# cokwa/bitHTM

Measured on AMD Instinct MI355X. Metric: HTM timesteps/sec (SP + TM, learning on), 65536 cols x 32 cells, higher is better.
Workload: dtype u32 bit-packed / f64 + f32 permanences; 1 GPU; configs[2]: 65536 columns x 32 cells, SP + TM learning on, 1 MI355X; input_dim=1024, column_dim=65536, cell_dim=32, active_columns=1311, patterns=50, pretrain_steps=500, segments=96476, segment_slots=128, hip_graph=True, hip_graph_requested=True, pipelined=True, repetitions=15, streamed_calls=True

## Files before the change

bithtm_amd/_lib.py:

```python

import ctypes as C
import os

HERE = os.path.dirname(os.path.abspath(__file__))
LIB_PATH = os.path.join(HERE, "libbithtm_hip.so")
ABI_VERSION = 4


class HtmConfig(C.Structure):
    _fields_ = [
        ("struct_bytes", C.c_uint32), ("device", C.c_int32),
        ("input_dim", C.c_int32), ("column_dim", C.c_int32), ("cell_dim", C.c_int32),
        ("active_columns", C.c_int32), ("enable_sp", C.c_int32), ("enable_tm", C.c_int32),
        ("sp_permanence_threshold", C.c_double), ("sp_delta_on", C.c_double), ("sp_delta_off", C.c_double),
        ("boost_coefficient", C.c_float), ("duty_momentum", C.c_float), ("duty_increment", C.c_float),
        ("tm_learn_active", C.c_double), ("tm_learn_inactive", C.c_double),
        ("tm_punish_active", C.c_double), ("tm_punish_inactive", C.c_double),
        ("tm_learn_prune", C.c_int32), ("tm_punish_prune", C.c_int32),
        ("tm_permanence_initial", C.c_float), ("tm_permanence_threshold", C.c_float),
        ("segment_activation_threshold", C.c_int32), ("segment_matching_threshold", C.c_int32),
        ("segment_sampling_synapses", C.c_int32),
        ("segment_capacity", C.c_int32), ("segment_capacity_local", C.c_int32), ("segment_slots", C.c_int32),
        ("seed", C.c_uint32), ("shard_rank", C.c_int32), ("shard_world", C.c_int32), ("use_caller_stream", C.c_int32),
        ("stream", C.c_void_p),
# ... 11 lines not shown
    ]


class HtmStepRecord(C.Structure):
    _fields_ = [(name, C.c_int32) for name in (
        "active_columns", "bursting_columns", "predicted_columns_before", "predicted_columns", "active_cells", "winner_cells",
        "segments", "new_segments")]


class HtmRunRecord(C.Structure):
    _fields_ = [("struct_bytes", C.c_uint32), ("records", C.c_void_p), ("active_column", C.c_void_p), ("column_prediction", C.c_void_p)]


class HtmSpRunRecord(C.Structure):
    _fields_ = [("struct_bytes", C.c_uint32), ("active_column", C.c_void_p), ("active_overlap", C.c_void_p), ("active_boosted", C.c_void_p)]


class HtmScalarField(C.Structure):
    _fields_ = [("minimum", C.c_double), ("scale", C.c_double)] + [(name, C.c_int32) for name in (
        "offset", "bits", "width", "buckets", "periodic", "reserved")]


class HtmLiveRow(C.Structure):
    _fields_ = HtmStepRecord._fields_ + [("step_index", C.c_int64), ("capacity_error", C.c_int32), ("reserved", C.c_int32)]


class HtmLikelihoodConfig(C.Structure):
    _fields_ = [("struct_bytes", C.c_uint32)] + [(name, C.c_int32) for name in (
        "learning_period", "estimation_samples", "history", "averaging_window", "reestimation_period")]


LIKELIHOOD_CHUNK = 512

F_ACTIVE_COLUMN, F_OVERLAPS, F_BOOSTED, F_DUTY_CYCLE, F_CELL_ACTIVATION, F_CELL_PREDICTION = 1, 2, 3, 4, 5, 6
F_WINNER_WORDS, F_BURSTING, F_WINNER_CELL, F_SEG_CELL, F_SEG_NSYN, F_SEG_PRESYN, F_SEG_PERM = 7, 8, 9, 10, 11, 12, 13
F_SEGCOUNT, F_SEG_POTENTIAL, F_MATCH_SEGMENT, F_MATCH_INFO, F_MATCH_JITTER, F_CELL_MAX_JITTER = 14, 15, 16, 17, 18, 19
F_SEG_GID = 20
F_RECYCLABLE_COUNTS = 21
PLAN_GRAPH, PLAN_PIPELINED, PLAN_LEAN, PLAN_SCAN_LARGE = 1, 2, 4, 8
SP_OVERLAP, SP_BOOST, SP_SELECT, SP_ACTIVE, SP_LEARN, SP_DUTY, SP_COMMIT = 1, 2, 3, 4, 5, 6, 7

EXPORTS = {
    "htm_abi_version": (C.c_int, []),
    "htm_create": (C.c_int, [C.POINTER(HtmConfig), C.POINTER(C.c_void_p)]),
    "htm_destroy": (None, [C.c_void_p]),
    "htm_last_error": (C.c_char_p, [C.c_void_p]),
    "htm_sp_set_permanence": (C.c_int, [C.c_void_p, C.c_void_p, C.c_int32, C.c_int32]),
    "htm_set_epsilon": (C.c_int, [C.c_void_p, C.c_float]),
    "htm_sp_get_permanence": (C.c_int, [C.c_void_p, C.c_void_p, C.c_int32, C.c_int32]),
    "htm_step": (C.c_int, [C.c_void_p, C.c_void_p, C.c_int32]),
    "htm_sp_step": (C.c_int, [C.c_void_p, C.c_void_p, C.c_int32]),
    "htm_sp_phase": (C.c_int, [C.c_void_p, C.c_int32, C.c_void_p, C.c_int64]),
    "htm_tm_step": (C.c_int, [C.c_void_p, C.c_void_p, C.c_int32, C.c_int32, C.c_int32]),
    "htm_tm_update": (C.c_int, [C.c_void_p, C.c_void_p, C.c_void_p, C.c_void_p, C.c_int32, C.c_void_p]),
    "htm_tm_scan": (C.c_int, [C.c_void_p, C.c_void_p]),
    "htm_tm_run": (C.c_int, [C.c_void_p, C.c_void_p, C.c_int32, C.c_int32, C.c_int32, C.c_int32, C.c_int32, C.POINTER(HtmRunRecord)]),
    "htm_sp_run": (C.c_int, [C.c_void_p, C.c_void_p, C.c_int32, C.c_int32, C.c_int32, C.c_int32, C.POINTER(HtmSpRunRecord)]),
    "htm_run": (C.c_int, [C.c_void_p, C.c_void_p, C.c_int32, C.c_int32, C.c_int32, C.c_int32]),
    "htm_prepare": (C.c_int, [C.c_void_p, C.c_void_p, C.c_int32, C.c_int32, C.c_int32, C.c_int32]),
    "htm_run_recorded": (C.c_int, [C.c_void_p, C.c_void_p, C.c_int32, C.c_int32, C.c_int32, C.c_int32, C.POINTER(HtmRunRecord)]),
    "htm_prepare_recorded": (C.c_int, [C.c_void_p, C.c_void_p, C.c_int32, C.c_int32, C.c_int32, C.c_int32]),
    "htm_reset": (C.c_int, [C.c_void_p]),
    "htm_set_run_resets": (C.c_int, [C.c_void_p, C.c_void_p, C.c_int32]),
    "htm_predicted_input": (C.c_int, [C.c_void_p, C.c_void_p]),
    "htm_set_run_predicted_input": (C.c_int, [C.c_void_p, C.c_void_p]),
    "htm_graph_count": (C.c_int, [C.c_void_p]),
    "htm_run_plan": (C.c_int, [C.c_void_p, C.c_int32, C.c_int32]),
    "htm_bank_upload": (C.c_int, [C.c_void_p, C.c_void_p, C.c_int32, C.POINTER(C.c_void_p)]),
    "htm_shard_record_bytes": (C.c_int64, [C.c_void_p]),
    "htm_shard_begin": (C.c_int, [C.c_void_p, C.c_void_p, C.c_int32, C.c_void_p, C.c_int32, C.c_void_p]),
    "htm_shard_finish": (C.c_int, [C.c_void_p, C.c_void_p, C.c_int32]),
    "htm_shard_unique_id": (C.c_int, [C.c_void_p]),
    "htm_shard_comm_init": (C.c_int, [C.c_void_p, C.c_void_p]),
    "htm_shard_step": (C.c_int, [C.c_void_p, C.c_void_p, C.c_int32, C.c_void_p, C.c_int32]),
    "htm_shard_comm_size": (C.c_int, [C.c_void_p]),
    "htm_shard_graph_ok": (C.c_int, [C.c_void_p]),
    "htm_shard_run": (C.c_int, [C.c_void_p, C.c_void_p, C.c_int32, C.c_int32, C.c_int32, C.c_int32]),
    "htm_shard_group_run": (C.c_int, [C.POINTER(C.c_void_p), C.c_int32, C.POINTER(C.c_void_p), C.c_int32, C.c_int32, C.c_int32, C.c_int32]),
    "htm_rccl_selftest": (C.c_int, [C.c_int32]),
    "htm_keyed_draws": (C.c_int, [C.c_uint32, C.c_int32, C.c_uint32, C.c_void_p, C.c_void_p, C.c_int64, C.c_void_p]),
    "htm_shard_group_step": (C.c_int, [C.POINTER(C.c_void_p), C.c_int32, C.POINTER(C.c_void_p), C.c_int32, C.c_void_p, C.c_int32]),
    "htm_populate": (C.c_int, [C.c_void_p, C.c_int64, C.c_int64, C.c_int32, C.c_int32, C.c_double, C.c_double, C.c_uint32]),
    "htm_sync": (C.c_int, [C.c_void_p]),
    "htm_get_stream": (C.c_int, [C.c_void_p, C.POINTER(C.c_void_p)]),
    "htm_get_info": (C.c_int, [C.c_void_p, C.POINTER(HtmInfo)]),
    "htm_read": (C.c_int64, [C.c_void_p, C.c_int32, C.c_void_p, C.c_int64]),
    "htm_read_rows": (C.c_int64, [C.c_void_p, C.c_int32, C.c_int64, C.c_int64, C.c_void_p, C.c_int64]),
    "htm_import_begin": (C.c_int, [C.c_void_p, C.c_int64]),
    "htm_write": (C.c_int, [C.c_void_p, C.c_int32, C.c_void_p, C.c_int64]),
    "htm_import_commit": (C.c_int, [C.c_void_p, C.c_int32, C.c_int32, C.c_int32, C.c_int32, C.c_int32]),
    "htm_profile": (C.c_int, [C.c_void_p, C.c_int32]),
    "htm_profile_read": (C.c_int, [C.c_void_p, C.c_int32, C.POINTER(C.c_char_p), C.POINTER(C.c_double),
                                   C.POINTER(C.c_int64)]),
    "htm_trace_read": (C.c_int64, [C.c_void_p, C.c_void_p, C.c_int64]),
    "htm_group_create": (C.c_int, [C.POINTER(C.c_void_p), C.c_int32, C.POINTER(C.c_void_p)]),
    "htm_group_destroy": (None, [C.c_void_p]),
    "htm_group_last_error": (C.c_char_p, [C.c_void_p]),
    "htm_group_run": (C.c_int, [C.c_void_p, C.POINTER(C.c_void_p), C.c_int32, C.c_int32, C.c_int32, C.c_int32, C.POINTER(HtmRunRecord)]),
    "htm_group_step": (C.c_int, [C.c_void_p, C.c_void_p, C.c_int32, C.POINTER(HtmRunRecord)]),
    "htm_create_view": (C.c_int, [C.c_void_p, C.POINTER(C.c_void_p)]),
    "htm_device_bytes": (C.c_int64, [C.c_void_p]),
    "htm_view_sync": (C.c_int, [C.c_void_p, C.c_void_p]),
    "htm_bank_rows": (C.c_int, [C.c_void_p, C.c_void_p, C.c_int32, C.c_int64, C.c_int32, C.c_void_p]),
    "htm_pack_columns": (C.c_int, [C.c_void_p, C.c_void_p, C.c_int32, C.c_int32, C.c_int32, C.c_void_p, C.c_int32, C.c_int32]),
    "htm_encode_votes": (C.c_int, [C.c_void_p, C.c_int32, C.c_int32, C.c_void_p, C.c_int32, C.c_int32]),
    "htm_set_run_feedback": (C.c_int, [C.c_void_p, C.c_void_p, C.c_int32, C.c_int32, C.c_int32]),
    "htm_bank_noise": (C.c_int, [C.c_void_p, C.c_void_p, C.c_int32, C.c_void_p, C.c_int32, C.c_uint32, C.c_int32, C.c_uint32, C.c_uint32,
                                 C.c_void_p, C.c_void_p]),
    "htm_bank_encode": (C.c_int, [C.c_void_p, C.POINTER(HtmScalarField), C.c_int32, C.c_void_p, C.c_int32, C.c_void_p, C.c_int32, C.c_int32]),
    "htm_decode_votes": (C.c_int, [C.c_void_p, C.POINTER(HtmScalarField), C.c_int32, C.c_void_p, C.c_int32, C.c_void_p]),
    "htm_predicted_value": (C.c_int, [C.c_void_p, C.POINTER(HtmScalarField), C.c_int32, C.c_void_p]),
    "htm_live_tick": (C.c_int, [C.c_void_p, C.c_void_p, C.POINTER(HtmScalarField), C.c_int32, C.c_void_p, C.c_void_p, C.c_int32, C.c_int32,
                                C.c_void_p, C.c_void_p, C.c_void_p]),
    "htm_live_reset": (C.c_int, [C.c_void_p, C.c_void_p]),
    "htm_likelihood_create": (C.c_int, [C.c_void_p, C.POINTER(HtmLikelihoodConfig), C.c_void_p, C.c_int32, C.POINTER(C.c_void_p)]),
    "htm_likelihood_destroy": (None, [C.c_void_p]),
    "htm_likelihood_update": (C.c_int, [C.c_void_p, C.c_void_p, C.POINTER(C.c_void_p), C.c_int32, C.c_void_p]),
    "htm_likelihood_reset": (C.c_int, [C.c_void_p, C.c_void_p, C.c_void_p]),
    "htm_likelihood_state_bytes": (C.c_int64, [C.c_void_p]),
    "htm_likelihood_export": (C.c_int, [C.c_void_p, C.c_void_p, C.c_void_p, C.c_int64]),
    "htm_likelihood_import": (C.c_int, [C.c_void_p, C.c_void_p, C.c_void_p, C.c_int64]),
    "htm_likelihood_tick": (C.c_int, [C.c_void_p, C.c_void_p, C.POINTER(HtmScalarField), C.c_int32, C.c_void_p, C.c_void_p, C.c_int32, C.c_int32,
                                      C.c_void_p, C.c_void_p, C.c_void_p, C.c_void_p, C.c_void_p]),
}

HIP_EXPORTS = {
    "hipSetDevice": (C.c_int, [C.c_int]),
    "hipMalloc": (C.c_int, [C.POINTER(C.c_void_p), C.c_size_t]),
    "hipFree": (C.c_int, [C.c_void_p]),
    "hipMemcpy": (C.c_int, [C.c_void_p, C.c_void_p, C.c_size_t, C.c_int]),
    "hipGetErrorString": (C.c_char_p, [C.c_int]),
    "hipStreamCreateWithFlags": (C.c_int, [C.POINTER(C.c_void_p), C.c_uint]),
    "hipStreamDestroy": (C.c_int, [C.c_void_p]),
}
HIP_MEMCPY_HOST_TO_DEVICE = 1
HIP_MEMCPY_DEVICE_TO_HOST = 2

_lib = None


def load():
    global _lib
    if _lib is not None:
        return _lib
    path = os.environ.get("BITHTM_LIBRARY") or LIB_PATH
    if not os.path.exists(path):
        raise ImportError(
            f"{path} is missing: the HIP extension is not built. Run `python -m bithtm_amd.build` "
            "(or __graft_entry__.build()). There is no CPU fallback.")
    try:
        lib = C.CDLL(path)
    except OSError as e:
        raise ImportError(f"cannot load {path}: {e}. There is no CPU fallback.") from e
    for name, (restype, argtypes) in list(EXPORTS.items()) + list(HIP_EXPORTS.items()):
        fn = getattr(lib, name)
        fn.restype = restype
        fn.argtypes = argtypes
    if lib.htm_abi_version() != ABI_VERSION:
        raise ImportError(f"{path}: ABI version {lib.htm_abi_version()} != {ABI_VERSION}; rebuild")
    _lib = lib
    return lib
```

bithtm_amd/csrc/htm_dev.h:

```cpp
#ifndef BITHTM_HTM_DEV_H
#define BITHTM_HTM_DEV_H

typedef unsigned long long u64;

#define SEL_MAX_PASSES 6
#define SEL_DIGIT 12
#define SEL_BINS 4096
#define HIST_REP 4
#define SEL_COARSE 64
#define COARSE_REP 16
#define COARSE_STRIDE 1024
#define FAN_COUNTERS 16
#define FAN_STRIDE 32
#define HIST0_FINE (HIST_REP * SEL_BINS)
#define HIST0_PAR (HIST0_FINE + COARSE_REP * COARSE_STRIDE)
#define RB 512
#define SCAN_SEGS 64
#define DEAD_CAP 256
#define SHARD_HOT_KEYS 4
#define CAND_CAP 256
#define WIN_LDS 4096
#define MAX_SLOTS 512
#define SYN_CONNECTED 0x80000000u
#define SYN_CELL 0x7FFFFFFF
#define SEG_BUSY 0x40000000
#define EPS32 1e-8f

#define KEY_SHIFT 3
__device__ __forceinline__ u64 select_key_bits(u64 bits) { return bits ? (bits - ((u64)(1023 - 150) << 52)) << KEY_SHIFT : 0ull; }
__device__ __forceinline__ u64 select_key(double boosted) { return select_key_bits((u64)__double_as_longlong(boosted)); }

#define WIN_COARSE 31
#define WIN_FINE 7
#define WIN_BINS (2 + (WIN_COARSE << WIN_FINE))
#define WIN_LOWBITS (52 - WIN_FINE)
static_assert(WIN_BINS <= SEL_BINS, "the window's bins fit the select histogram");
__host__ __device__ __forceinline__ uint32_t win_bin(u64 key, uint32_t base) {
    const uint32_t c = (uint32_t)(key >> 52);
    if (c < base) return 0u;
    const uint32_t o = c - base;
    return o >= WIN_COARSE ? 1u + (WIN_COARSE << WIN_FINE) : 1u + ((o << WIN_FINE) | ((uint32_t)(key >> WIN_LOWBITS) & ((1u << WIN_FINE) - 1u)));
}
__host__ __device__ __forceinline__ uint32_t win_base_for(u64 kth_key) {
    const uint32_t c = (uint32_t)(kth_key >> 52);
    return c > WIN_COARSE / 2 ? min(c - WIN_COARSE / 2, 4096u - WIN_COARSE) : 0u;
}

__host__ __device__ __forceinline__ uint32_t win_base_global(u64 kth_key) { return win_base_for(kth_key); }

__host__ __device__ __forceinline__ int sel_shift(int pass) { return pass < 5 ? 52 - SEL_DIGIT * pass : 0; }
__host__ __device__ __forceinline__ int sel_bits(int pass) { return pass < 5 ? SEL_DIGIT : 4; }

struct Counters {
    uint32_t step[2];
    int32_t S;
    int32_t n_win[2];
    int32_t has_winner[2];
    int32_t has_distal;
    uint32_t cm_dense_step;
    int32_t n_active_cells;
    alignas(128) int32_t n_work[2];
    int32_t n_bind[2];
    alignas(128) int32_t n_work_last;
    int32_t sel_fallbacks;
    int32_t cand_exact;
    int32_t hot_selects;
    int32_t sel_zooms;
    uint32_t emit_epoch;
    int32_t n_un;
    int32_t n_recycled, n_new, S_old;
    int32_t L;
    int32_t n_lfree;
    int32_t error;
    u64 sel_prefix[2];
    uint32_t sel_krem[2];
    uint32_t sel_win[2];
    uint32_t sel_win_global;
    u64 sel_pass_prefix[2][SEL_MAX_PASSES + 1];
    uint32_t sel_pass_krem[2][SEL_MAX_PASSES + 1];
};

struct Dev {
    int I, W, W4, Ipad, C, K, k, E, Scap, work_cap, sel_passes, colwords, low_zero, cand_d, cand_pairwise, cand_others, cand_speculate, cand_take_all, cand_zoom, poll_delay;
    int win_offset;
    int cls_rows_max;
    int LK, KP, WPC;
    int world, c0, c1;
    int sel_lo, sel_hi, sel_k;
    int Lcap, n_cand;
    int hot_budget, hot_target;
    int cand_cap;
    double sp_thr, sp_don, sp_doff;
    float coef, mom, dinc;
    double lrn_act, lrn_inact, pun_act, pun_inact;
    int lrn_prune, pun_prune;
    float perm_init, perm_thr;
    float eps;
    int act_thr, match_thr, sample;
    uint32_t seed;
    double *perm;
    uint32_t *mask;
    float *duty;
    int *overlap[2];
    double *boosted[2];
    u64 *key[2];
    uint32_t *hist;
    uint32_t *hist0;
    uint32_t *sel_blk;
    uint32_t *sel_rec;
    int *active_cols[2];
    uint32_t *input_stage;
    uint32_t *act[2];
    uint32_t *pred[2];
    uint32_t *win[2];
    uint32_t *colbits[2];
    int *winners[2];
    uint8_t *bursting;
    int *actw_id;
    uint32_t *winw_idx;
    uint8_t *actcnt;
    uint32_t *act_list;
    uint16_t *col_rank[2];
    uint32_t *unacc_word;
    uint32_t *fan;
    int *unacc_list;
    int *seg_cell;
    int *seg_nsyn;
    int *presyn;
    float *sperm;
    int *segcount;
    uint32_t *cellmax[2];
    uint32_t *match_bits[2];
    uint32_t *seg_info;
    float *seg_jit;
    uint32_t *work;
    int *recyc_cnt;
    int *recyc_cnt2;
    int *recyc_need;
    int *seg_gid;
    int *g2l;
    uint32_t *dead_bits;
    int *lfree;
    int *asg_gid;
    int *cand_cols;
    int *dead_list;
    const uint32_t *punish;
    unsigned char *send;
    Counters *ctr;
    unsigned long long *trace;
    uint32_t trace_until;
};

__device__ __forceinline__ int lane_id() { return threadIdx.x & 63; }
__device__ __forceinline__ u64 lanemask_lt() { return (1ull << lane_id()) - 1ull; }

__device__ __forceinline__ uint32_t wave_incl_scan(uint32_t v) {
    uint32_t t = v;
    t += (uint32_t)__builtin_amdgcn_update_dpp(0, (int)v, 0x111, 0xf, 0xf, false);
    t += (uint32_t)__builtin_amdgcn_update_dpp(0, (int)v, 0x112, 0xf, 0xf, false);
    t += (uint32_t)__builtin_amdgcn_update_dpp(0, (int)v, 0x113, 0xf, 0xf, false);
    t += (uint32_t)__builtin_amdgcn_update_dpp(0, (int)t, 0x114, 0xf, 0xe, false);
    t += (uint32_t)__builtin_amdgcn_update_dpp(0, (int)t, 0x118, 0xf, 0xc, false);
    t += (uint32_t)__builtin_amdgcn_update_dpp(0, (int)t, 0x142, 0xa, 0xf, false);
    t += (uint32_t)__builtin_amdgcn_update_dpp(0, (int)t, 0x143, 0xc, 0xf, false);
    return t;
}

__device__ __forceinline__ uint32_t wave_sum(uint32_t v) { return (uint32_t)__builtin_amdgcn_readlane((int)wave_incl_scan(v), 63); }

#ifdef BITHTM_BISECT_A
__device__ __forceinline__ uint32_t wave_read(uint32_t v, int src) { return (uint32_t)__shfl((int)v, src); }
__device__ __forceinline__ int wave_read(int v, int src) { return __shfl(v, src); }
#else
__device__ __forceinline__ uint32_t wave_read(uint32_t v, int src) { return (uint32_t)__builtin_amdgcn_readlane((int)v, src); }
__device__ __forceinline__ int wave_read(int v, int src) { return __builtin_amdgcn_readlane(v, src); }
#endif
__device__ __forceinline__ u64 wave_read(u64 v, int src) {
#ifdef BITHTM_BISECT_A
    return ((u64)(uint32_t)__shfl((int)(v >> 32), src) << 32) | (uint32_t)__shfl((int)(uint32_t)v, src);
#endif
    return ((u64)(uint32_t)__builtin_amdgcn_readlane((int)(v >> 32), src) << 32) | (uint32_t)__builtin_amdgcn_readlane((int)(uint32_t)v, src);
}

template <typename Op>
__device__ __forceinline__ u64 wave_reduce64(u64 v, u64 ident, Op op) {
    const int il = (int)(uint32_t)ident, ih = (int)(ident >> 32);
#define BITHTM_DPP64(src, ctrl, rm, bm) \
    (((u64)(uint32_t)__builtin_amdgcn_update_dpp(ih, (int)((src) >> 32), ctrl, rm, bm, false) << 32) | \
     (uint32_t)__builtin_amdgcn_update_dpp(il, (int)(uint32_t)(src), ctrl, rm, bm, false))
    u64 t = v;
    t = op(t, BITHTM_DPP64(v, 0x111, 0xf, 0xf));
    t = op(t, BITHTM_DPP64(v, 0x112, 0xf, 0xf));
    t = op(t, BITHTM_DPP64(v, 0x113, 0xf, 0xf));
    t = op(t, BITHTM_DPP64(t, 0x114, 0xf, 0xe));
    t = op(t, BITHTM_DPP64(t, 0x118, 0xf, 0xc));
    t = op(t, BITHTM_DPP64(t, 0x142, 0xa, 0xf));
    t = op(t, BITHTM_DPP64(t, 0x143, 0xc, 0xf));
#undef BITHTM_DPP64
    return wave_read(t, 63);
}

__device__ __forceinline__ int group8_sum_first(int v) {
    int t = v;
    t += __builtin_amdgcn_update_dpp(0, v, 0x101, 0xf, 0xf, false);
    t += __builtin_amdgcn_update_dpp(0, v, 0x102, 0xf, 0xf, false);
    t += __builtin_amdgcn_update_dpp(0, v, 0x103, 0xf, 0xf, false);
    t += __builtin_amdgcn_update_dpp(0, t, 0x104, 0xf, 0xf, false);
    return t;
}

__device__ __forceinline__ int group8_sum_all(int v) {
    v += __builtin_amdgcn_update_dpp(0, v, 0xB1, 0xf, 0xf, false);
    v += __builtin_amdgcn_update_dpp(0, v, 0x4E, 0xf, 0xf, false);
    v += __builtin_amdgcn_update_dpp(0, v, 0x141, 0xf, 0xf, false);
    return v;
}

__device__ __forceinline__ void store_through(int *p, int v) { asm volatile("global_store_dword %0, %1, off sc0 sc1" ::"v"(p), "v"(v) : "memory"); }
__device__ __forceinline__ void store_through(float *p, float v) { asm volatile("global_store_dword %0, %1, off sc0 sc1" ::"v"(p), "v"(v) : "memory"); }

__device__ __forceinline__ void lds_barrier() { asm volatile("s_waitcnt lgkmcnt(0)\n\ts_barrier" ::: "memory"); }

template <typename Op>
__device__ __forceinline__ float half_reduce(float v, float ident, Op op) {
    const int id = __float_as_int(ident);
#define BITHTM_DPPF(src, ctrl, rm, bm) __int_as_float(__builtin_amdgcn_update_dpp(id, __float_as_int(src), ctrl, rm, bm, false))
    float t = v;
    t = op(t, BITHTM_DPPF(v, 0x111, 0xf, 0xf));
    t = op(t, BITHTM_DPPF(v, 0x112, 0xf, 0xf));
    t = op(t, BITHTM_DPPF(v, 0x113, 0xf, 0xf));
    t = op(t, BITHTM_DPPF(t, 0x114, 0xf, 0xe));
    t = op(t, BITHTM_DPPF(t, 0x118, 0xf, 0xc));
    t = op(t, BITHTM_DPPF(t, 0x142, 0xa, 0xf));
// ... 77 lines not shown
```

bithtm_amd/csrc/htm_engine.hip:

```cpp

#include <hip/hip_runtime.h>
#include <hip/hip_ext.h>
#include <dlfcn.h>
#include <stdint.h>
#include <stdio.h>
#include <string.h>
#include <algorithm>
#include <cfloat>
#include <climits>
#include <cmath>
#include <chrono>
#include <map>
#include <mutex>
#include <string>
#include <tuple>
#include <type_traits>
#include <vector>

#include "../../include/bithtm_hip.h"
#include "htm_fexp.h"
#include "htm_rng.h"

#include "htm_dev.h"
#include "htm_sp_kernels.h"
#include "htm_tm_kernels.h"
#include "htm_pipeline.h"
#include "htm_record.h"
#include "htm_reset.h"
#include "htm_decode.h"
#include "htm_stack.h"
#include "htm_forecast.h"
#include "htm_noise.h"
#include "htm_group.h"
#include "htm_tm_feed.h"
#include "htm_sp_run.h"
#include "htm_fork.h"
#include "htm_scalar.h"
#include "htm_live.h"
#include "htm_likelihood.h"


struct ncclUniqueIdBytes { char internal[128]; };

static thread_local std::string g_create_error;
static int (*g_rccl_destroy)(void *) = nullptr;

struct Knobs {
    int graph_steps, eager_below;
    bool trace;
    uint32_t trace_until;
    int lean, lean2_classify, lean2_order, step_split, fuse_tm, shard_window, step_window, tail_rows, scan_large, scan_large_above, scan_dyn;
    int defer_tail, shared_scan, shared_members;
    int lean_overlap, lean_learn, lean_learn_large, lean_scan, lean_scan_large, scan_blocks, sel_launch_digits;
    int cand_d, cand_pairwise, cls_rows_max, win_offset, cand_zoom, cand_speculate, cand_take_all, poll_delay, cand_others;
};

struct Sizes {
    int G;
    int sp_blocks, sel_blocks, c256_blocks, s1024_blocks, scan_blocks, zero_blocks, cus;
    int lean_learn_blocks, lean_learn_blocks_large, lean_scan_blocks, lean_scan_blocks_large, lean_overlap_blocks, lean2_classify_blocks;
    int lean_resident_large;
    bool emit_fits, emit_fits_open;
    bool emit_fits_lean;
    int sel_passes_fused, sel_passes_full;
};

struct RunModes {
    bool recording, resetting, decoding, feeding;
    bool operator<(const RunModes &o) const { return std::tie(recording, resetting, decoding, feeding) < std::tie(o.recording, o.resetting, o.decoding, o.feeding); }
};

struct RunGraphKey {
    int p; RunModes modes; int learning; bool sp_done, next_sp, next_front, lean; int spec; bool large, emit_fused, wmode;
    int span; const void *bank; int n_inputs;
    auto tie() const { return std::tie(p, modes, learning, sp_done, next_sp, next_front, lean, spec, large, emit_fused, wmode, span, bank, n_inputs); }
    bool operator<(const RunGraphKey &o) const { return tie() < o.tie(); }
};

struct ShardGraphKey {
    int p, learning; bool front_done, front_next; int span, ranks, n_inputs; std::vector<std::tuple<int, bool, bool>> per_rank; const void *bank;
    auto tie() const { return std::tie(p, learning, front_done, front_next, span, ranks, n_inputs, per_rank, bank); }
    bool operator<(const ShardGraphKey &o) const { return tie() < o.tie(); }
};

struct TmRunGraphKey {
    int p; RunModes modes; int learning, spec; bool large; int span; const void *lists; int n_rows, n;
    auto tie() const { return std::tie(p, modes, learning, spec, large, span, lists, n_rows, n); }
    bool operator<(const TmRunGraphKey &o) const { return tie() < o.tie(); }
};

struct SpRunGraphKey {
    int p, learning; bool recording, emit_fused; int wmode, span; const void *bank; int n_inputs;
    auto tie() const { return std::tie(p, learning, recording, emit_fused, wmode, span, bank, n_inputs); }
    bool operator<(const SpRunGraphKey &o) const { return tie() < o.tie(); }
};

struct htm_handle {
    htm_config cfg;
    Dev d;
    Knobs knob;
    Sizes sz;
    int device;
    hipStream_t stream;
    bool own_stream;
    long long step_host;
    std::string err;
    std::vector<void *> allocs;
    int *d_cols_stage;
    int rank, world;
    const uint32_t *shard_bank;
    int shard_n_inputs = 1;
    bool shard_open;
    bool shard_graph_ok;
    int shard_front_wmode;
    std::map<ShardGraphKey, hipGraphExec_t> shard_graphs;
    void *rccl_comm;
    unsigned char *shard_send, *shard_recv;
    bool emit_fused, emit_fused_open;
    bool tail_pending;
    int tail_p;
    bool window_known;
    int seg_hint;
    int *seg_pinned;
    const uint32_t *ahead_bank;
    int ahead_n_inputs, ahead_learning;
    bool ahead_lean;
    int phase_active;
    bool phase_wide;
    bool import_keep;
    bool phase_open;
    RecDev *d_rec;
    const uint32_t *reset_bits;
    int reset_n;
    ResetDev *d_reset;
    int32_t *pin_out;
    PinDev *d_pin;
    int32_t *d_pin_buf;
    int32_t *d_value_out;
    uint32_t *feed_bank;
    int feed_n;
    FeedDev *d_feed;
    int32_t *d_feed_votes;
    std::map<RunGraphKey, hipGraphExec_t> graphs;
    std::map<TmRunGraphKey, hipGraphExec_t> tm_graphs;
    std::map<SpRunGraphKey, hipGraphExec_t> sp_graphs;
    SpRecDev *d_sp_rec;
    std::vector<int> imp_pot, imp_match_seg;
    std::vector<int> imp_seg_cell, imp_seg_nsyn, imp_presyn;
    std::vector<float> imp_perm;
    std::vector<uint32_t> imp_match_info;
    std::vector<float> imp_match_jit;
    bool profile;
    hipEvent_t prof_last;
    std::vector<hipEvent_t> prof_all;
    std::vector<std::string> prof_names;
    std::vector<std::vector<std::pair<hipEvent_t, hipEvent_t>>> prof_events;
    std::vector<double> prof_ms;
    std::vector<long long> prof_n;
    std::vector<void *> weight_allocs;
    struct HtmShared *shared;
    bool is_view;
    long long seen_wgen;
    uint32_t dense_step;
    int64_t own_bytes;
};

struct HtmShared {
    std::vector<void *> allocs;
    hipStream_t stream;
    bool own_stream;
    htm_handle *parent;
    int refs;
    long long wgen;
};
static std::mutex g_shared_mutex;

static std::mutex g_registry_mutex;
static std::vector<htm_handle *> g_registry;

static void refresh_exchange_mode(htm_handle *h) {
    bool solo = true;
    {
        std::lock_guard<std::mutex> lock(g_registry_mutex);
        for (const htm_handle *o : g_registry)
            if (o != h && o->device == h->device && o->stream != h->stream) solo = false;
    }
    h->emit_fused = h->sz.emit_fits && solo;
    h->emit_fused_open = h->sz.emit_fits_open && solo;
    h->d.sel_passes = h->emit_fused ? h->sz.sel_passes_fused : h->sz.sel_passes_full;
}

#define HIPCHK(h, call)                                                                          \
    do {                                                                                         \
        hipError_t e_ = (call);                                                                  \
        if (e_ != hipSuccess) {                                                                  \
            (h)->err = std::string(#call) + ": " + hipGetErrorString(e_);                        \
            return HTM_ERR_HIP;                                                                  \
        }                                                                                        \
    } while (0)

static bool sp_is_ahead(const htm_handle *h) { return h->ahead_bank != nullptr; }
#define REJECT_WHEN_AHEAD(h)                                                                                      \
    do {                                                                                                          \
        if (sp_is_ahead(h)) {                                                                                     \
            (h)->err = "the Spatial Pooler is ahead (htm_run ended with HTM_RUN_CONTINUE): continue with htm_run on the same bank"; \
            return HTM_ERR_STATE;                                                                                 \
        }                                                                                                         \
    } while (0)

static int launch_status(std::string &err) {
    const hipError_t e = hipGetLastError();
    if (e == hipSuccess) return HTM_OK;
    err = std::string("kernel launch: ") + hipGetErrorString(e);
    return HTM_ERR_HIP;
}

static void refresh_seg_hint(htm_handle *h) {
    if (h->seg_pinned) h->seg_hint = std::max(h->seg_hint, (int)*(volatile int *)h->seg_pinned);
}

static hipError_t hand_back_segments(htm_handle *h, const int32_t *count, hipStream_t stream) {
    return h->seg_pinned ? hipMemcpyAsync(h->seg_pinned, count, sizeof(int), hipMemcpyDeviceToHost, stream) : hipSuccess;
}

template <typename Key, typename Enqueue>
static hipGraphExec_t cached_graph(std::map<Key, hipGraphExec_t> &graphs, const Key &key, hipStream_t stream, std::string &err, Enqueue enqueue) {
    auto it = graphs.find(key);
    if (it != graphs.end()) return it->second;
    hipError_t e = hipStreamBeginCapture(stream, hipStreamCaptureModeThreadLocal);
    if (e != hipSuccess) { err = std::string("hipStreamBeginCapture: ") + hipGetErrorString(e); return nullptr; }
    const int rc = enqueue();
    hipGraph_t graph = nullptr;
    hipGraphExec_t exec = nullptr;
    e = hipStreamEndCapture(stream, &graph);
    if (rc) {
    } else if (e != hipSuccess || !graph) {
        err = std::string("hipStreamEndCapture: ") + hipGetErrorString(e);
    } else if ((e = hipGraphInstantiate(&exec, graph, nullptr, nullptr, 0)) != hipSuccess) {
        err = std::string("hipGraphInstantiate: ") + hipGetErrorString(e);
        exec = nullptr;
    }
    if (graph) hipGraphDestroy(graph);
    if (exec) graphs.emplace(key, exec);
    return exec;
}

template <typename T>
// ... 127 lines not shown
        launch_scan(h, p, scan_lds(d, 1) <= 64 * 1024);
    }
}

static void flush_tail(htm_handle *h) {
    if (!h->tail_pending) return;
    h->tail_pending = false;
    hipSetDevice(h->device);
    enqueue_tm_tail(h, h->tail_p);
}

static decltype(&k_learn_scan_tail<1>) const kt_learn_scan_tail[4] = {k_learn_scan_tail<1>, k_learn_scan_tail<2>, k_learn_scan_tail<4>, k_learn_scan_tail<8>};

static void enqueue_tm(htm_handle *h, int n_active, int learning, int want_winner, int p,
                       const uint32_t *bank, int n_inputs, bool sp_rows, int front_wmode = -1, bool defer_tail = false) {
    Dev &d = h->d;
    const int n_cls = learning ? kClassifyBlocks : 0;
    const bool fuse = tm_tail_fused(h);
    int n_sp_rows = (sp_rows && learning && h->cfg.enable_sp) ? d.k : 0;
    const int n_tail_rows = (fuse && h->world == 1 && h->knob.tail_rows && !defer_tail) ? n_sp_rows : 0;
    if (n_tail_rows) n_sp_rows = 0;
    const int n_duty = h->world > 1 ? (d.c1 - d.c0 + 255) / 256 : 0;
    LAUNCH(h, "tm_mid", k_mid_rows, 1 + n_cls + n_sp_rows + n_duty + h->sz.zero_blocks, 256, d, p, n_active, want_winner, learning, n_cls, bank, n_inputs, n_sp_rows, 0, n_duty);
    if (defer_tail) { h->tail_pending = true; h->tail_p = p; return; }
    if (fuse && (front_wmode >= 0 || n_tail_rows)) {
        const int epl = learn_epl(d), n_learn = h->sz.lean_learn_blocks, n_scan = h->sz.lean_scan_blocks, spec = scan_spec_blocks(h);
        const size_t lds = std::max(std::max(learn_lds(epl, 256), scan_lds(d, 1)), (size_t)SEL_BINS * 4);
        const int grid = n_learn + n_scan + (n_tail_rows ? n_tail_rows : h->sz.lean_overlap_blocks);
        const char *name = n_tail_rows ? "tm_learn+tm_scan+sp_learn" : "tm_learn+tm_scan+shard_overlap";
        LAUNCH_ON(h, h->stream, lds, name, kt_learn_scan_tail[epl_slot(d)], grid, 256, d, p, n_learn, n_scan, spec, bank, n_inputs, h->sz.G, front_wmode, n_tail_rows);
        return;
    }
    enqueue_tm_tail(h, p);
    if (front_wmode >= 0)
        LAUNCH(h, "shard_overlap", k_shard_overlap, h->sz.sp_blocks, RB, d, bank, n_inputs, h->sz.G, p, front_wmode, 1);
}

struct StepPlan { bool sp_done, next_sp, next_front; };

static bool can_pipeline(const htm_handle *h) {
    return h->cfg.enable_sp && h->cfg.enable_tm && h->world == 1 && h->emit_fused_open && h->d.sel_passes == 2;
}

static bool can_lean(const htm_handle *h) {
    return h->knob.lean && can_pipeline(h) && scan_lds(h->d, 1) <= 64 * 1024 && h->sz.emit_fits_lean;
}

static decltype(&k_learn_scan_emit<1, 6>) const kt_lse_large[4] = {k_learn_scan_emit<1, 4, false>, k_learn_scan_emit<2, 4, false>,
                                                                   k_learn_scan_emit<4, 4, false>, k_learn_scan_emit<8, 4, false>};
static decltype(&k_learn_scan_emit<1, 6>) const kt_lse_tab[4] = {k_learn_scan_emit<1, 6, true>, k_learn_scan_emit<2, 6, true>,
                                                                 k_learn_scan_emit<4, 6, true>, k_learn_scan_emit<8, 6, true>};
static decltype(&k_learn_scan_emit<1, 6>) lse_kernel(const Dev &d, int form) {
    return (form == LSE_TAB ? kt_lse_tab : form == LSE_LARGE ? kt_lse_large : kt_lse_plain)[epl_slot(d)];
}

static int lse_form(const htm_handle *h) { return scan_pool_is_large(h) ? LSE_LARGE : lean_tab(h->d) ? LSE_TAB : LSE_PLAIN; }

static void launch_learn_scan_emit(htm_handle *h, int p, int n_emit) {
    Dev &d = h->d;
    const int epl = learn_epl(d);
    const size_t lds = std::max(std::max(learn_lds(epl, 256), lean_scan_lds(d)), sizeof(EmitShared));
    const bool large = scan_pool_is_large(h), dyn = large && h->knob.scan_dyn > 0;
    const int n_learn = dyn ? h->sz.lean_learn_blocks_large : h->sz.lean_learn_blocks;
    int n_scan = large ? h->sz.lean_scan_blocks_large : h->sz.lean_scan_blocks;
    if (dyn) n_scan = std::max(64, h->sz.lean_resident_large - n_emit - n_learn);
    const int grid = n_emit + n_learn + n_scan;
    if (large && !dyn) n_scan = -n_scan;
    const int spec = dyn ? 0 : scan_spec_blocks(h);
    const char *lse_name = large ? "tm_learn+tm_scan_large+sp_emit" : "tm_learn+tm_scan+sp_emit";
    LAUNCH_ON(h, h->stream, lds, lse_name, lse_kernel(d, lse_form(h)), grid, 256, d, p, n_emit, n_learn, n_scan, spec);
}

static int lean2_classify_blocks(const htm_handle *h, int learning) {
    if (!learning) return 0;
    return scan_pool_is_large(h) && !h->knob.lean2_classify ? std::max(h->sz.lean2_classify_blocks, 192) : h->sz.lean2_classify_blocks;
}

static void enqueue_lean(htm_handle *h, int p, int learning, const uint32_t *bank, int n_inputs, StepPlan plan) {
    Dev &d = h->d;
    const int n_act = (d.k * d.KP + 255) / 256, n_rows = learning ? d.k : 0;
    const int n_cls = learning ? kClassifyBlocks : 0, n_ov = plan.next_sp ? h->sz.lean_overlap_blocks : 0;
    if (h->knob.lean == 2) {
        const int n_cls2 = lean2_classify_blocks(h, learning);
        const int n_duty = n_ov ? 0 : h->sz.c256_blocks, n_clear = d.WPC * h->sz.c256_blocks;
        LAUNCH_ON(h, h->stream, (size_t)SEL_BINS * 4, "tm_activate+tm_mid+sp_learn+sp_overlap", k_act_mid_rows,
                  n_act + 1 + n_cls2 + n_rows + n_ov + n_duty + n_clear + h->sz.zero_blocks, 256, d, p, d.k, n_act, learning, n_cls2, bank, n_inputs, n_rows, h->sz.G, n_ov,
                  n_duty, n_clear, h->knob.lean2_order);
    } else {
        LAUNCH(h, "tm_activate+sp_learn", k_act_rows, n_act + n_rows + (1 + d.WPC) * h->sz.c256_blocks, 256, d, p, d.k, n_act, bank, n_inputs, n_rows, h->sz.c256_blocks);
        LAUNCH_ON(h, h->stream, (size_t)SEL_BINS * 4, "tm_mid+sp_overlap", k_mid_overlap, 1 + n_cls + n_ov + h->sz.zero_blocks, 256, d, p, d.k, 1, learning, n_cls,
                  bank, n_inputs, h->sz.G, n_ov);
    }
    launch_learn_scan_emit(h, p, plan.next_sp ? h->sz.c256_blocks : 0);
}

static decltype(&k_learn_overlap<1>) const kt_learn_overlap[4] = {k_learn_overlap<1>, k_learn_overlap<2>, k_learn_overlap<4>, k_learn_overlap<8>};
static decltype(&k_scan_sel<true, 1>) const kt_scan_sel[4] = {k_scan_sel<true, 1>, k_scan_sel<false, 1>, k_scan_sel<true, 6>, k_scan_sel<false, 6>};

static void enqueue_pipelined(htm_handle *h, int p, int learning, const uint32_t *bank, int n_inputs, StepPlan plan) {
    Dev &d = h->d;
    const int n_cls = learning ? kClassifyBlocks : 0;
    const int n_emit = plan.next_sp ? h->sz.c256_blocks : 0;
    LAUNCH_ON(h, h->stream, sizeof(EmitShared), "tm_activate+sp_emit", k_open_emit, n_emit + (d.k * d.KP + 255) / 256, 256, d, p, n_emit, d.k);
    const int n_rows = (plan.next_sp && learning) ? d.k : 0, n_duty = plan.next_sp ? h->sz.c256_blocks : 0;
    LAUNCH(h, "tm_mid+sp_learn", k_mid_rows, 1 + n_cls + n_rows + n_duty + h->sz.zero_blocks, 256, d, p, d.k, 1, learning, n_cls, bank, n_inputs, n_rows, 1, n_duty);
    LAUNCH_ON(h, h->stream, std::max(learn_lds(learn_epl(d)), (size_t)SEL_BINS * 4), "tm_learn+sp_overlap", kt_learn_overlap[epl_slot(d)],
              kLearnBlocks + (plan.next_front ? h->sz.sp_blocks : 0), RB, d, p, kLearnBlocks, bank, n_inputs, h->sz.G, p, 2);
    const bool use_lds = scan_lds(d, 1) <= 64 * 1024, large = scan_pool_is_large(h);
    const int n_sel = plan.next_front ? 64 : 0, n_clear = plan.next_sp ? h->sz.c256_blocks : 0;
    LAUNCH_ON(h, h->stream, std::max(scan_lds(d, use_lds), sizeof(SelShared)), large ? "tm_scan_large+sp_select" : "tm_scan+sp_select",
              kt_scan_sel[scan_slot(large, use_lds)], h->sz.scan_blocks + n_sel + n_clear, 256, d, p, n_sel, n_clear, p, scan_spec_blocks(h));
}

static void enqueue_cold_start(htm_handle *h, const uint32_t *bank, int n_inputs, int learning, StepPlan plan) {
    Dev &d = h->d;
    const int p = (int)(h->step_host & 1);
    if (plan.sp_done || !plan.next_sp) return;
    const int wmode = step_wmode(h);
    if (can_lean(h)) {
        enqueue_sp_front(h, bank, n_inputs, p, wmode);
        enqueue_sp_back(h, bank, n_inputs, p, 1, 0, false, wmode);
        return;
    }
    enqueue_sp_front(h, bank, n_inputs, p, wmode);
    enqueue_sp_back(h, bank, n_inputs, p, 1, EMIT_DUTY | EMIT_CLEAR, learning != 0, wmode);
    LAUNCH(h, "sp_overlap", k_sp_overlap, h->sz.sp_blocks, RB, d, bank, n_inputs, h->sz.G, p, p ^ 1, 1, 0);
    LAUNCH(h, "sp_select", k_sel_pass, h->sz.sel_blocks, RB, d, 1, p ^ 1);
}

static int reset_blocks(const Dev &d) { return std::max(1, std::min(1024, (d.C * d.KP + 255) / 256)); }

static void enqueue_run_reset(htm_handle *h, RunModes m, int p) {
    if (m.resetting) LAUNCH(h, "tm_reset", k_tm_reset, reset_blocks(h->d), 256, h->d, p, h->d_reset, m.recording ? h->d_rec : nullptr, 0u);
}

static void enqueue_rest(htm_handle *h, RunModes m, int p, const uint32_t *bank, int n_inputs, int learning, StepPlan plan) {
    enqueue_run_reset(h, m, p);
    if ((plan.sp_done || plan.next_sp) && can_lean(h)) {
        enqueue_lean(h, p, learning, bank, n_inputs, plan);
    } else if (plan.sp_done || plan.next_sp) {
        enqueue_pipelined(h, p, learning, bank, n_inputs, plan);
    } else {
        enqueue_sp_back(h, bank, n_inputs, p, 1, EMIT_ALL, false, step_wmode(h));
        enqueue_tm(h, h->d.k, learning, 1, p, bank, n_inputs, true);
    }
}

static int rec_blocks(const Dev &d) { return std::max(REC_BLOCKS_MIN, (d.k + 255) / 256); }

static void enqueue_record(htm_handle *h, RunModes m, int p) {
    if (m.recording) LAUNCH(h, "record", k_rec_step, rec_blocks(h->d), 256, h->d, p, h->d_rec);
}

static void enqueue_decode(htm_handle *h, RunModes m, int p) {
    if (m.decoding) LAUNCH(h, "predicted_input", k_pin_step, pin_blocks(h->d.C), 256, h->d, p, (const PinDev *)h->d_pin);
}

static bool decode_unpipelined(const htm_handle *h) { return h->pin_out && !can_lean(h); }

static void enqueue_feed(htm_handle *h, RunModes m, int p) {
    if (!m.feeding) return;
    LAUNCH(h, "feedback_votes", k_feed_votes, pin_blocks(h->d.C), 256, h->d, p, (const FeedDev *)h->d_feed);
    LAUNCH(h, "feedback_encode", k_feed_step, 1, ENC_THREADS, h->d, p, (const FeedDev *)h->d_feed);
}

static int pin_begin_blocks(int n, int I) { return (int)std::max<size_t>(1, std::min<size_t>(1024, ((size_t)n * I + 255) / 256)); }

static void enqueue_step_outputs(htm_handle *h, RunModes m, int p) {
    enqueue_record(h, m, p);
    enqueue_decode(h, m, p);
    enqueue_feed(h, m, p);
}

static int enqueue_step(htm_handle *h, RunModes m, const uint32_t *bank, int n_inputs, int learning, StepPlan plan, const uint32_t *host_input = nullptr) {
    const int p = (int)(h->step_host & 1);
    if (!plan.sp_done && !plan.next_sp) enqueue_sp_front(h, bank, n_inputs, p, step_wmode(h), host_input);
    enqueue_cold_start(h, bank, n_inputs, learning, plan);
    enqueue_rest(h, m, p, bank, n_inputs, learning, plan);
    enqueue_step_outputs(h, m, p);
    h->step_host += 1;
    return launch_status(h->err);
}

extern "C" int htm_abi_version(void) { return BITHTM_ABI_VERSION; }

extern "C" const char *htm_last_error(const htm_handle *h) { return h ? h->err.c_str() : g_create_error.c_str(); }

extern "C" void htm_destroy(htm_handle *h) {
    if (!h) return;
    {
        std::lock_guard<std::mutex> lock(g_registry_mutex);
        g_registry.erase(std::remove(g_registry.begin(), g_registry.end(), h), g_registry.end());
    }
    hipSetDevice(h->device);
    hipStreamSynchronize(h->stream);
    for (auto &kv : h->graphs) hipGraphExecDestroy(kv.second);
    for (auto &kv : h->shard_graphs) hipGraphExecDestroy(kv.second);
    for (auto &kv : h->tm_graphs) hipGraphExecDestroy(kv.second);
    for (auto &kv : h->sp_graphs) hipGraphExecDestroy(kv.second);
    for (auto &v : h->prof_events)
        for (auto &pr : v) { hipEventDestroy(pr.first); hipEventDestroy(pr.second); }
    for (hipEvent_t e : h->prof_all) hipEventDestroy(e);
    if (h->rccl_comm && g_rccl_destroy) g_rccl_destroy(h->rccl_comm);
    for (void *p : h->allocs) hipFree(p);
    for (void *p : h->weight_allocs) hipFree(p);
    if (h->seg_pinned) hipHostFree(h->seg_pinned);
    if (h->own_stream) hipStreamDestroy(h->stream);
    if (HtmShared *sh = h->shared) {
        bool last;
        {
            std::lock_guard<std::mutex> lock(g_shared_mutex);
            if (sh->parent == h) sh->parent = nullptr;
            last = --sh->refs == 0;
        }
        if (last) {
            for (void *p : sh->allocs) hipFree(p);
            if (sh->own_stream) hipStreamDestroy(sh->stream);
            delete sh;
        }
    }
    delete h;
}

static int fail_create(htm_handle *h, const std::string &msg, int code) {
    g_create_error = msg;
    if (h) { h->err = msg; htm_destroy(h); }
    return code;
}

static int alloc_weights(htm_handle *h) {
    Dev &d = h->d;
    const htm_config *cfg = &h->cfg;
    const size_t C = d.C;
    int rc = 0;
    if (cfg->enable_sp) {
        rc |= dalloc_weights(h, &d.perm, C * d.Ipad);
        rc |= dalloc_weights(h, &d.mask, C * d.W);
    }
    if (cfg->enable_tm) {
        const size_t S = d.Lcap, E = d.E, KP = d.KP;
        rc |= dalloc_weights(h, &d.seg_cell, S);
        rc |= dalloc_weights(h, &d.seg_nsyn, S);
        rc |= dalloc_weights(h, &d.presyn, S * E);
        rc |= dalloc_weights(h, &d.sperm, S * E);
        rc |= dalloc_weights(h, &d.segcount, C * KP);
    }
    return rc;
}

static int alloc_stream_state(htm_handle *h) {
    Dev &d = h->d;
    const htm_config *cfg = &h->cfg;
    const int world = h->world;
    int rc = 0;
    const size_t C = d.C, k = d.k;
    rc |= dalloc(h, &d.ctr, 1);
    rc |= dalloc(h, &d.active_cols[0], k + 8);
    rc |= dalloc(h, &d.active_cols[1], k + 8);
    if (cfg->enable_sp) {
        rc |= dalloc(h, &d.duty, C);
        for (int q = 0; q < 2; ++q) {
            rc |= dalloc(h, &d.overlap[q], C);
            rc |= dalloc(h, &d.boosted[q], C);
            rc |= dalloc(h, &d.key[q], C);
        }
        rc |= dalloc(h, &d.hist, (size_t)2 * SEL_MAX_PASSES * SEL_BINS);
        rc |= dalloc(h, &d.hist0, (size_t)2 * HIST0_PAR);
        rc |= dalloc(h, &d.sel_blk, (C + 255) / 256);
        rc |= dalloc(h, &d.sel_rec, (C + 255) / 256 * 32);
        rc |= dalloc(h, &d.input_stage, (size_t)d.W);
    }
    if (cfg->enable_tm) {
        const size_t S = d.Lcap, G = d.Scap;
        const size_t KP = d.KP, WPC = d.WPC;
        for (int q = 0; q < 2; ++q) {
            rc |= dalloc(h, &d.act[q], C * WPC);
            rc |= dalloc(h, &d.pred[q], C * WPC);
            rc |= dalloc(h, &d.winners[q], k * KP);
        }
        rc |= dalloc(h, &d.win[0], C * WPC);
        rc |= dalloc(h, &d.win[1], C * WPC);
        d.colwords = (int)((C + 63) / 64) * 2;
        const size_t colwords_padded = (size_t)((C + 255) / 256) * 8;
        rc |= dalloc(h, &d.colbits[0], colwords_padded);
        rc |= dalloc(h, &d.colbits[1], colwords_padded);
        rc |= dalloc(h, &d.bursting, k);
        rc |= dalloc(h, &d.actw_id, k * WPC + 8);
        rc |= dalloc(h, &d.winw_idx, k * WPC + 8);
        rc |= dalloc(h, &d.actcnt, k * WPC + 8);
        rc |= dalloc(h, &d.act_list, k * WPC + 16);
        rc |= dalloc(h, &d.col_rank[0], colwords_padded);
        rc |= dalloc(h, &d.col_rank[1], colwords_padded);
        rc |= dalloc(h, &d.unacc_word, k * WPC + 8);
        rc |= dalloc(h, &d.fan, (size_t)2 * FAN_COUNTERS * FAN_STRIDE);
        rc |= dalloc(h, &d.unacc_list, k * KP);
        for (int q = 0; q < 2; ++q) {
            rc |= dalloc(h, &d.cellmax[q], C * KP);
            rc |= dalloc(h, &d.match_bits[q], (S + 255) / 256 * 8);
        }
        rc |= dalloc(h, &d.seg_info, S);
        rc |= dalloc(h, &d.seg_jit, S);
        rc |= dalloc(h, &d.work, (size_t)d.work_cap);
        rc |= dalloc(h, &d.recyc_cnt, (G + 1023) / 1024);
        rc |= dalloc(h, &d.recyc_cnt2, ((G + 1023) / 1024 + 1023) / 1024 + 1);
        rc |= dalloc(h, &d.recyc_need, 2 * k * KP);
        rc |= dalloc(h, &d.dead_list, (size_t)1 + DEAD_CAP);
        if (world > 1) {
            rc |= dalloc(h, &d.seg_gid, S);
            rc |= dalloc(h, &d.g2l, G);
            rc |= dalloc(h, &d.dead_bits, (G + 31) / 32 + 32);
            rc |= dalloc(h, &d.lfree, S);
            rc |= dalloc(h, &d.asg_gid, k * 32);
            rc |= dalloc(h, &d.cand_cols, (size_t)d.n_cand + 8);
            if (!rc && (hipMemsetAsync(d.seg_gid, 0xFF, S * 4, h->stream) != hipSuccess ||
                        hipMemsetAsync(d.g2l, 0xFF, G * 4, h->stream) != hipSuccess)) { h->err = "hipMemsetAsync failed"; rc = HTM_ERR_HIP; }
        }
        rc |= dalloc(h, &h->d_cols_stage, k);
    }
    if (h->knob.trace) rc |= dalloc(h, &d.trace, (size_t)8 * 4096 * 2);
    return rc;
}

static const char *env_str(const char *name) { return getenv(name); }
static int env_int(const char *name, int dflt, int lo = INT_MIN, int hi = INT_MAX) {
    const char *e = env_str(name);
    return e ? std::max(lo, std::min(hi, atoi(e))) : dflt;
}
static int env_flag(const char *name, int dflt) {
    const char *e = env_str(name);
    return e ? atoi(e) != 0 : dflt;
}

static Knobs read_knobs() {
    Knobs k;
    k.graph_steps = env_int("BITHTM_GRAPH_STEPS", 16, 1, 256);
    k.eager_below = env_int("BITHTM_EAGER_BELOW", 64, 0);
    k.trace = env_str("BITHTM_TRACE") != nullptr;
    const char *until = env_str("BITHTM_TRACE_UNTIL");
    k.trace_until = until ? (uint32_t)strtoul(until, nullptr, 10) : 0xFFFFFFFFu;
    k.lean = env_int("BITHTM_LEAN", 2, 0, 2);
    k.lean2_classify = env_int("BITHTM_LEAN2_CLASSIFY", 0, 1);
    k.step_split = env_flag("BITHTM_STEP_SPLIT", 1);
    {
        const char *e = env_str("BITHTM_LEAN2_ORDER");
        const int o = e ? (int)strtol(e, nullptr, 16) : 0x0312;
        int seen = 0, pos[4] = {-1, -1, -1, -1};
        for (int i = 0; i < 4; ++i) { const int r = (o >> (4 * (3 - i))) & 15; if (r < 4) { seen |= 1 << r; pos[r] = i; } }
        k.lean2_order = (o >= 0 && o <= 0x3333 && seen == 15 && pos[0] < pos[1]) ? o : 0x0312;
    }
    k.fuse_tm = env_flag("BITHTM_FUSE_TM", 1);
    k.shard_window = env_flag("BITHTM_SHARD_WINDOW", 1);
    k.scan_large = env_int("BITHTM_SCAN_LARGE", -1);
    k.scan_large_above = env_int("BITHTM_SCAN_LARGE_ABOVE", 3 * 1536 * SCAN_SEGS, 0);
    k.step_window = env_flag("BITHTM_STEP_WINDOW", 1);
    k.tail_rows = env_flag("BITHTM_TAIL_ROWS", 1);
    k.scan_dyn = env_flag("BITHTM_SCAN_DYN", 1);
    k.defer_tail = env_flag("BITHTM_DEFER_TAIL", 1);
    k.shared_scan = env_flag("BITHTM_SHARED_SCAN", 0);
    k.shared_members = env_int("BITHTM_SHARED_SCAN_MEMBERS", 0, 0);
    k.lean_overlap = env_int("BITHTM_LEAN_OVERLAP", 0, 1);
    k.lean_learn = env_int("BITHTM_LEAN_LEARN", 0, 1);
    k.lean_learn_large = env_int("BITHTM_LEAN_LEARN_LARGE", 0, 1);
    k.lean_scan = env_int("BITHTM_LEAN_SCAN", 0, 1);
    k.lean_scan_large = env_int("BITHTM_LEAN_SCAN_LARGE", 0, 1);
    k.scan_blocks = env_int("BITHTM_SCAN_BLOCKS", 0, 1);
    k.sel_launch_digits = env_int("BITHTM_SEL_LAUNCH_DIGITS", -1, 0);
    k.cand_d = env_int("BITHTM_CAND_D", CAND_D, 0, CAND_D);
    k.cand_pairwise = env_int("BITHTM_CAND_PAIRWISE", CAND_PAIRWISE, 0);
    k.cls_rows_max = env_int("BITHTM_CLASSIFY_WORDS_ABOVE", -1, 0);
    k.win_offset = env_int("BITHTM_SEL_WINDOW_OFFSET", 0, 0);
    k.cand_zoom = env_int("BITHTM_CAND_ZOOM", -1);
    k.cand_speculate = env_flag("BITHTM_CAND_SPECULATE", 1);
    k.cand_take_all = env_flag("BITHTM_CAND_TAKE_ALL", 1);
    k.poll_delay = env_int("BITHTM_POLL_DELAY", 7, 0, 64);
    k.cand_others = env_int("BITHTM_CAND_OTHERS", CAND_OTHERS, 0, CAND_OTHERS);
    return k;
}

static void size_launches(htm_handle *h) {
    Dev &d = h->d;
    const Knobs &k = h->knob;
    Sizes &z = h->sz;
    z.G = 1;
    while (z.G < d.W4 && z.G < 64) z.G <<= 1;
    const int rows_per_block = (RB / 64) * 4 * (64 / z.G);
    z.sp_blocks = std::max(1, std::min((d.c1 - d.c0 + rows_per_block - 1) / rows_per_block, 256));
    z.sel_blocks = std::max(1, std::min((d.sel_hi - d.sel_lo + RB - 1) / RB, 128));
    z.c256_blocks = (d.sel_hi - d.sel_lo + 255) / 256;
    z.s1024_blocks = std::max(1, (d.Scap + 1023) / 1024);
    z.scan_blocks = std::max(1, std::min((d.Lcap + SCAN_SEGS - 1) / SCAN_SEGS, 2048));
    if (z.scan_blocks > 256) z.scan_blocks = (z.scan_blocks + 255) & ~255;
    z.zero_blocks = std::max(1, std::min((d.Lcap / 128 + 4095) / 4096, 1024));
    z.lean_overlap_blocks = k.lean_overlap ? k.lean_overlap : z.sp_blocks * (RB / 256);
    z.lean_learn_blocks = k.lean_learn ? k.lean_learn : 512;
    z.lean_learn_blocks_large = k.lean_learn_large ? k.lean_learn_large : k.lean_learn ? z.lean_learn_blocks : 768;
    z.lean_scan_blocks = k.lean_scan ? k.lean_scan : (z.scan_blocks > 512 ? std::max(256, (z.scan_blocks * 3 / 8 + 255) & ~255) : z.scan_blocks);
    z.lean_scan_blocks_large = k.lean_scan_large ? k.lean_scan_large : k.lean_scan ? z.lean_scan_blocks : z.scan_blocks;
    if (k.scan_blocks) z.scan_blocks = k.scan_blocks;
    hipDeviceProp_t prop;
    const bool have_prop = hipGetDeviceProperties(&prop, h->device) == hipSuccess;
    z.cus = have_prop ? prop.multiProcessorCount : 256;
    int B = 0;
    while ((1ll << B) <= (long long)d.I) ++B;
    const int informative = std::min(64, 64 - (29 - B) - KEY_SHIFT);
    d.sel_passes = std::max(1, std::min(SEL_MAX_PASSES, (informative + SEL_DIGIT - 1) / SEL_DIGIT));
    d.low_zero = 64 - informative;
    int per_cu_emit = 0, per_cu_open = 0;
    if (have_prop && hipOccupancyMaxActiveBlocksPerMultiprocessor(&per_cu_emit, (const void *)k_sp_emit, 256, 0) == hipSuccess &&
        hipOccupancyMaxActiveBlocksPerMultiprocessor(&per_cu_open, (const void *)k_open_emit, 256, sizeof(EmitShared)) == hipSuccess) {
        z.emit_fits = z.c256_blocks <= std::min(1024, per_cu_emit * z.cus);
        z.emit_fits_open = z.emit_fits && z.c256_blocks + (d.k * d.KP + 255) / 256 <= std::min(1024, per_cu_open * z.cus);
        int per_cu_lean = 1 << 30;
        z.lean_resident_large = 1 << 30;
        const size_t lean_lds = std::max(std::max(learn_lds(learn_epl(d), 256), lean_scan_lds(d)), sizeof(EmitShared));
        bool asked = h->cfg.enable_tm && z.emit_fits && lean_lds <= 64 * 1024;
        for (int form = LSE_TAB; asked && form <= LSE_LARGE; ++form) {
            if (form == LSE_TAB && !lean_tab(d)) continue;
            int per_cu = 0;
            asked = hipOccupancyMaxActiveBlocksPerMultiprocessor(&per_cu, (const void *)lse_kernel(d, form), 256, lean_lds) == hipSuccess;
            per_cu_lean = std::min(per_cu_lean, per_cu);
            if (asked && form == LSE_LARGE) z.lean_resident_large = per_cu * z.cus;
        }
        z.emit_fits_lean = asked && z.c256_blocks <= std::min(1024, per_cu_lean * z.cus);
        if (z.lean_resident_large == (1 << 30)) z.lean_resident_large = 4 * z.cus;
    } else {
        (void)hipGetLastError();
        z.emit_fits = z.emit_fits_open = z.emit_fits_lean = false;
        z.lean_resident_large = 1024;
    }
    if (k.lean2_classify) {
        z.lean2_classify_blocks = k.lean2_classify;
    } else {
        int per_cu = 0, resident = 1536;
        if (have_prop && hipOccupancyMaxActiveBlocksPerMultiprocessor(&per_cu, (const void *)k_act_mid_rows, 256, (size_t)SEL_BINS * 4) == hipSuccess)
            resident = per_cu * z.cus;
        else
            (void)hipGetLastError();
        const int others = (d.k * d.KP + 255) / 256 + z.lean_overlap_blocks + d.k + 1;
        const int room = (resident - others) & ~7;
        z.lean2_classify_blocks = room >= 128 ? std::min(kClassifyBlocks, room) : 32;
    }
    z.sel_passes_full = d.sel_passes;
    z.sel_passes_fused = std::min(d.sel_passes, 2);
    if (k.sel_launch_digits >= 0) z.sel_passes_fused = std::max(2, std::min(d.sel_passes, k.sel_launch_digits));
}

extern "C" int htm_create(const htm_config *cfg, htm_handle **out) {
    if (!cfg || !out) return fail_create(nullptr, "htm_create: null argument", HTM_ERR_ARGUMENT);
    if (cfg->struct_bytes != sizeof(htm_config)) return fail_create(nullptr, "htm_create: htm_config size mismatch (ABI)", HTM_ERR_ARGUMENT);
    if (cfg->column_dim < 1 || cfg->active_columns < 1 || cfg->active_columns > cfg->column_dim)
        return fail_create(nullptr, "htm_create: need 1 <= active_columns <= column_dim", HTM_ERR_ARGUMENT);
    if (cfg->enable_sp && cfg->input_dim < 1) return fail_create(nullptr, "htm_create: input_dim < 1", HTM_ERR_ARGUMENT);
    if (cfg->enable_tm) {
        if (cfg->cell_dim < 1 || cfg->cell_dim > 64) return fail_create(nullptr, "htm_create: cell_dim must be in 1..64", HTM_ERR_ARGUMENT);
        if (cfg->segment_slots < 64 || cfg->segment_slots > MAX_SLOTS || cfg->segment_slots % 64)
            return fail_create(nullptr, "htm_create: segment_slots must be a multiple of 64 in 64..512", HTM_ERR_ARGUMENT);
        if (cfg->segment_capacity < 1) return fail_create(nullptr, "htm_create: segment_capacity < 1", HTM_ERR_ARGUMENT);
        if (cfg->segment_sampling_synapses < 1 || cfg->segment_sampling_synapses > 64)
            return fail_create(nullptr, "htm_create: segment_sampling_synapses must be in 1..64", HTM_ERR_ARGUMENT);
        if (cfg->segment_activation_threshold < cfg->segment_matching_threshold)
            return fail_create(nullptr, "htm_create: activation threshold < matching threshold", HTM_ERR_ARGUMENT);
        if ((long long)cfg->column_dim * (cfg->cell_dim > 32 ? 64 : 32) > 0x7FFFFFFFLL) return fail_create(nullptr, "htm_create: column_dim too large", HTM_ERR_ARGUMENT);
    }
    if (!cfg->enable_sp && !cfg->enable_tm) return fail_create(nullptr, "htm_create: nothing enabled", HTM_ERR_ARGUMENT);
    const int world = cfg->shard_world > 1 ? cfg->shard_world : 1;
    if (world > 1) {
        if (!cfg->enable_sp || !cfg->enable_tm) return fail_create(nullptr, "htm_create: a sharded handle needs SP and TM", HTM_ERR_ARGUMENT);
        if (cfg->cell_dim > 32) return fail_create(nullptr, "htm_create: a sharded handle takes cell_dim up to 32 (the exchange record carries one 32-bit word per column)", HTM_ERR_ARGUMENT);
        if (world > 64) return fail_create(nullptr, "htm_create: at most 64 shards", HTM_ERR_ARGUMENT);
        if (cfg->shard_rank < 0 || cfg->shard_rank >= world) return fail_create(nullptr, "htm_create: shard_rank out of range", HTM_ERR_ARGUMENT);
        if (cfg->column_dim % (world * 64)) return fail_create(nullptr, "htm_create: column_dim must be a multiple of 64 * shard_world", HTM_ERR_ARGUMENT);
    }

    htm_handle *h = new htm_handle();
    h->cfg = *cfg;
    h->device = cfg->device;
// ... 277 lines not shown
    const int rc = launch_status(view->err);
    if (rc) return rc;
    refresh_seg_hint(source);
    view->step_host = source->step_host;
    view->seg_hint = source->seg_hint;
    if (view->seg_pinned) *view->seg_pinned = source->seg_hint;
    view->window_known = source->window_known;
    view->seen_wgen = source->is_view ? source->seen_wgen : wgen;
    view->dense_step = source->dense_step;
    return HTM_OK;
}

extern "C" int htm_bank_rows(htm_handle *h, const uint32_t *device_bank, int32_t bank_rows, int64_t first_step, int32_t n, uint32_t *device_dst) {
    if (!h || !device_bank || !device_dst) return HTM_ERR_ARGUMENT;
    if (bank_rows < 1 || first_step < 0 || n < 0 || n > bank_rows) { h->err = "htm_bank_rows: bank_rows >= 1, first_step >= 0 and 0 <= n <= bank_rows"; return HTM_ERR_ARGUMENT; }
    if ((((uintptr_t)device_bank | (uintptr_t)device_dst) & 15) != 0) { h->err = "htm_bank_rows: the bank and the destination must be 16-byte aligned"; return HTM_ERR_ARGUMENT; }
    if (!h->cfg.enable_sp) { h->err = "htm_bank_rows: needs a handle with the device's own Spatial Pooler (its input rows are packed)"; return HTM_ERR_STATE; }
    if (n == 0) return HTM_OK;
    HIPCHK(h, hipSetDevice(h->device));
    LAUNCH(h, "bank_rows", k_bank_rows, n, 256, device_bank, (int)bank_rows, (int)(first_step % bank_rows), h->d.W4, device_dst);
    return launch_status(h->err);
}

extern "C" int htm_set_epsilon(htm_handle *h, float epsilon) {
    if (!h) return HTM_ERR_ARGUMENT;
    if (h) flush_tail(h);
    if (!(epsilon > 0.f) || epsilon > 1.f) { h->err = "htm_set_epsilon: need 0 < epsilon <= 1"; return HTM_ERR_ARGUMENT; }
    REJECT_WHEN_AHEAD(h);
    if (epsilon == h->d.eps) return HTM_OK;
    HIPCHK(h, hipSetDevice(h->device));
    HIPCHK(h, hipStreamSynchronize(h->stream));
    for (auto &kv : h->graphs) hipGraphExecDestroy(kv.second);
    h->graphs.clear();
    h->d.eps = epsilon;
    return HTM_OK;
}

extern "C" int htm_get_stream(htm_handle *h, void **stream) {
    if (!h || !stream) return HTM_ERR_ARGUMENT;
    *stream = (void *)h->stream;
    return HTM_OK;
}

extern "C" int htm_sync(htm_handle *h) {
    if (!h) return HTM_ERR_ARGUMENT;
    if (h) flush_tail(h);
    HIPCHK(h, hipSetDevice(h->device));
    const auto t0 = std::chrono::steady_clock::now();
    for (;;) {
        const hipError_t e = hipStreamQuery(h->stream);
        if (e == hipSuccess) return HTM_OK;
        if (e != hipErrorNotReady) { h->err = std::string("hipStreamQuery: ") + hipGetErrorString(e); return HTM_ERR_HIP; }
        if (std::chrono::steady_clock::now() - t0 > std::chrono::milliseconds(2)) break;
    }
    HIPCHK(h, hipStreamSynchronize(h->stream));
    return HTM_OK;
}

static int check_rows(htm_handle *h, const void *rows, int row_begin, int row_count) {
    if (!h) return HTM_ERR_ARGUMENT;
    if (!h->cfg.enable_sp) { h->err = "handle has no Spatial Pooler"; return HTM_ERR_STATE; }
    if (!rows || row_begin < 0 || row_count < 0 || row_begin + (long long)row_count > h->d.C) {
        h->err = "permanence rows out of range";
        return HTM_ERR_ARGUMENT;
    }
    return 0;
}

extern "C" int htm_sp_set_permanence(htm_handle *h, const double *rows, int32_t row_begin, int32_t row_count) {
    if (h) REFUSE_ON_VIEW(h, "htm_sp_set_permanence");
    if (h) flush_tail(h);
    if (h) weights_touched(h);
    int rc = check_rows(h, rows, row_begin, row_count);
    if (rc) return rc;
    REJECT_WHEN_AHEAD(h);
    if (row_count == 0) return HTM_OK;
    Dev &d = h->d;
    HIPCHK(h, hipSetDevice(h->device));
    HIPCHK(h, hipMemcpy2DAsync(d.perm + (size_t)row_begin * d.Ipad, (size_t)d.Ipad * 8, rows, (size_t)d.I * 8,
                               (size_t)d.I * 8, (size_t)row_count, hipMemcpyHostToDevice, h->stream));
    const long long waves = (long long)row_count * (d.Ipad / 64);
    const int blocks = (int)std::min<long long>((waves + 3) / 4, 8192);
    hipLaunchKernelGGL(k_sp_build_mask, dim3(blocks), dim3(256), 0, h->stream, d, row_begin, row_count);
    HIPCHK(h, hipStreamSynchronize(h->stream));
    return HTM_OK;
}

extern "C" int htm_sp_get_permanence(htm_handle *h, double *rows, int32_t row_begin, int32_t row_count) {
    if (h) flush_tail(h);
    int rc = check_rows(h, rows, row_begin, row_count);
    if (rc) return rc;
    REJECT_WHEN_AHEAD(h);
    if (row_count == 0) return HTM_OK;
    Dev &d = h->d;
    HIPCHK(h, hipSetDevice(h->device));
    HIPCHK(h, hipMemcpy2DAsync(rows, (size_t)d.I * 8, d.perm + (size_t)row_begin * d.Ipad, (size_t)d.Ipad * 8,
                               (size_t)d.I * 8, (size_t)row_count, hipMemcpyDeviceToHost, h->stream));
    HIPCHK(h, hipStreamSynchronize(h->stream));
    return HTM_OK;
}

static int close_open_phases(htm_handle *h) {
    if (!h->phase_open) return 0;
    const int p = (int)(h->step_host & 1);
    if (h->cfg.enable_sp) HIPCHK(h, hipMemsetAsync(h->d.hist0 + (size_t)p * HIST0_PAR, 0, (size_t)HIST0_PAR * 4, h->stream));
    h->phase_open = false;
    h->phase_active = 0;
    h->phase_wide = false;
    return 0;
}

static int stage_input(htm_handle *h, const uint32_t *packed_input) {
    Dev &d = h->d;
    const int words = (d.I + 31) / 32;
    HIPCHK(h, hipMemcpyAsync(d.input_stage, packed_input, (size_t)words * 4, hipMemcpyHostToDevice, h->stream));
    return 0;
}

static decltype(&k_learn_scan_front<1>) const kt_learn_scan_front[4] = {k_learn_scan_front<1>, k_learn_scan_front<2>, k_learn_scan_front<4>, k_learn_scan_front<8>};

extern "C" int htm_step(htm_handle *h, const uint32_t *packed_input, int32_t learning) {
    if (!h || !packed_input) return HTM_ERR_ARGUMENT;
    REJECT_WHEN_AHEAD(h);
    if (!h->cfg.enable_sp || !h->cfg.enable_tm) { h->err = "htm_step needs a handle with SP and TM"; return HTM_ERR_STATE; }
    if (h->world > 1) { h->err = "sharded handle: use htm_shard_begin / htm_shard_finish"; return HTM_ERR_STATE; }
    HIPCHK(h, hipSetDevice(h->device));
    int rc = view_enter(h, learning);
    if (rc) return rc;
    if (learning) weights_touched(h);
    refresh_exchange_mode(h);
    rc = close_open_phases(h);
    if (rc) return rc;
    if (h->d.W > ARG_INPUT_WORDS) {
        flush_tail(h);
        rc = stage_input(h, packed_input);
        if (rc) return rc;
    }
    Dev &d = h->d;
    if (h->knob.defer_tail && d.W <= ARG_INPUT_WORDS && tm_tail_fused(h) && !h->profile) {
        const int p = (int)(h->step_host & 1), wmode = step_wmode(h);
        const bool ride_emit = h->knob.step_split && h->tail_pending && wmode && h->emit_fused && can_lean(h);
        bool emitted = false;
        if (ride_emit) {
            enqueue_sp_front(h, d.input_stage, 1, p, wmode, packed_input);
            h->tail_pending = false;
            launch_learn_scan_emit(h, h->tail_p, h->sz.c256_blocks);
            h->window_known = true;
            emitted = true;
        } else if (h->tail_pending) {
            PackedInputArg in;
            memset(&in, 0, sizeof(in));
            memcpy(in.w, packed_input, (size_t)((d.I + 31) / 32) * 4);
            const int epl = learn_epl(d), n_learn = h->sz.lean_learn_blocks, n_scan = h->sz.lean_scan_blocks, spec = scan_spec_blocks(h);
            const size_t lds = std::max(std::max(learn_lds(epl, 256), scan_lds(d, 1)), (size_t)(SEL_BINS + ARG_INPUT_WORDS) * 4);
            const int grid = n_learn + n_scan + h->sz.lean_overlap_blocks;
            h->tail_pending = false;
            LAUNCH_ON(h, h->stream, lds, "tm_learn+tm_scan+sp_overlap", kt_learn_scan_front[epl_slot(d)], grid, 256, d, h->tail_p, n_learn, n_scan, spec, in, h->sz.G, p, wmode);
            if (!wmode)
                for (int pass = 1; pass < d.sel_passes; ++pass) LAUNCH(h, "sp_select", k_sel_pass, h->sz.sel_blocks, RB, d, pass, p);
        } else {
            enqueue_sp_front(h, d.input_stage, 1, p, wmode, packed_input);
        }
        if (h->knob.step_split) {
            if (!emitted) enqueue_sp_back(h, d.input_stage, 1, p, 1, 0, false, wmode);
            const int lrn = learning ? 1 : 0;
            const int n_act = (d.k * d.KP + 255) / 256, n_rows = lrn ? d.k : 0;
            const int n_cls2 = lean2_classify_blocks(h, lrn);
            const int n_duty = h->sz.c256_blocks, n_clear = d.WPC * h->sz.c256_blocks;
            LAUNCH_ON(h, h->stream, 0, "tm_activate+tm_mid+sp_learn", k_act_mid_rows, n_act + 1 + n_cls2 + n_rows + n_duty + n_clear + h->sz.zero_blocks, 256,
                      d, p, d.k, n_act, lrn, n_cls2, d.input_stage, 1, n_rows, h->sz.G, 0, n_duty, n_clear, h->knob.lean2_order);
            h->tail_pending = true;
            h->tail_p = p;
        } else {
            enqueue_sp_back(h, d.input_stage, 1, p, 1, EMIT_ALL, false, wmode);
            enqueue_tm(h, d.k, learning ? 1 : 0, 1, p, d.input_stage, 1, true, -1, true);
        }
        h->step_host += 1;
        return launch_status(h->err);
    }
    flush_tail(h);
    return enqueue_step(h, RunModes{}, h->d.input_stage, 1, learning ? 1 : 0, StepPlan{false, false, false}, packed_input);
// ... 2521 lines not shown
```

bithtm_amd/csrc/htm_pipeline.h:

```cpp
#ifndef BITHTM_HTM_PIPELINE_H
#define BITHTM_HTM_PIPELINE_H

struct TraceScope {
    unsigned long long *t;
    __device__ TraceScope(const Dev &d, int slot) {
#if defined(BITHTM_LEARN_STAMPS) || defined(BITHTM_SCAN_STAMPS) || defined(BITHTM_EMIT_STAMPS) || defined(BITHTM_SHARD_STAMPS)
        t = nullptr;
        return;
#endif
        t = (d.trace && blockIdx.x < 4096 && d.ctr->step[slot >> 2] < d.trace_until) ? d.trace + ((size_t)slot * 4096 + blockIdx.x) * 2 : nullptr;
        if (t && threadIdx.x == 0) t[0] = wall_clock64();
    }
    __device__ ~TraceScope() { if (t && threadIdx.x == 0) t[1] = wall_clock64(); }
};

__global__ __launch_bounds__(256) void k_open_emit(Dev d, int p, int n_emit_blocks, int n_active) {
    TraceScope ts(d, 0 + 4 * p);
    if ((int)blockIdx.x < n_emit_blocks) {
        role_emit(d, p ^ 1, 1, 1, 0, blockIdx.x, n_emit_blocks, (EmitShared *)dyn_lds);
    } else {
        const int idx = ((int)blockIdx.x - n_emit_blocks) * tm_groups_per_block(d) + tm_group_of(d, threadIdx.x);
        const bool ok = idx < n_active;
        const int a = ok ? d.active_cols[p][idx] : 0;
        tm_activate_column(d, p, 1, ok, a, idx, tm_pred_words(d, p, ok, a));
    }
}

#ifndef BITHTM_MID_ROWS_WAVES
#define BITHTM_MID_ROWS_WAVES 8
#endif
__global__ __launch_bounds__(256, BITHTM_MID_ROWS_WAVES) void k_mid_rows(Dev d, int p, int n_active, int want_winner, int learning, int n_cls,
                                                  const uint32_t *__restrict__ bank, int n_inputs, int n_rows, int rows_ahead, int n_duty_blocks) {
    TraceScope ts(d, 1 + 4 * p);
    int b = blockIdx.x;
    if (b <= n_cls) {
        role_mid<256>(d, p, n_active, want_winner, learning, b, n_cls);
        return;
    }
    b -= 1 + n_cls;
    const int q = p ^ 1;
    if (b < n_rows) {
        role_sp_row<256>(d, rows_ahead ? q : p, bank, n_inputs, rows_ahead, b, threadIdx.x);
        return;
    }
    b -= n_rows;
    const int c = d.c0 + b * 256 + (int)threadIdx.x;
    if (b < n_duty_blocks) {
        if (c < d.c1) {
            float dc = d.duty[c] * d.mom;
            if ((d.colbits[rows_ahead ? q : p][c >> 5] >> (c & 31)) & 1u) dc = dc + d.dinc;
            d.duty[c] = dc;
        }
        return;
    }
    b -= n_duty_blocks;
    const int nz = (int)gridDim.x - 1 - n_cls - n_rows - n_duty_blocks;
    const int words4 = ((d.world > 1 ? d.ctr->L : d.ctr->S) + 127) >> 7;
    uint4 *mb = (uint4 *)d.match_bits[p];
    for (int i = b * 256 + (int)threadIdx.x; i < words4; i += nz * 256) mb[i] = make_uint4(0u, 0u, 0u, 0u);
}

template <int EPL>
__global__ __launch_bounds__(RB) void k_learn_overlap(Dev d, int p, int n_learn_blocks, const uint32_t *__restrict__ bank,
                                                        int n_inputs, int G, int sp, int step_offset) {
    TraceScope ts(d, 2 + 4 * p);
    if ((int)blockIdx.x < n_learn_blocks)
        role_learn<EPL, RB>(d, p, blockIdx.x, n_learn_blocks, (LearnShared<EPL, RB> *)dyn_lds);
    else
        role_overlap<RB>(d, bank, n_inputs, G, p, sp, step_offset, blockIdx.x - n_learn_blocks, gridDim.x - n_learn_blocks, (uint32_t *)dyn_lds);
}

template <bool use_lds, int MINW>
__global__ __launch_bounds__(256, MINW) void k_scan_sel(Dev d, int p, int n_sel_blocks, int n_clear_blocks, int sp, int n_spec) {
    TraceScope ts(d, 3 + 4 * p);
    int b = blockIdx.x;
    if (b < n_sel_blocks) {
        role_sel_pass<256>(d, 1, sp, b, n_sel_blocks, (SelShared *)dyn_lds);
        return;
    }
    b -= n_sel_blocks;
    if (b < n_clear_blocks) {
        const int q = p ^ 1;
        for (int c = b * 256 + (int)threadIdx.x; c < d.C * d.WPC; c += n_clear_blocks * 256) {
            d.act[q][c] = 0;
            d.win[q][c] = 0;
            d.pred[q][c] = 0;
        }
        return;
    }
    b -= n_clear_blocks;
    role_scan<256, use_lds, MINW == 1>(d, p, b, gridDim.x - n_sel_blocks - n_clear_blocks, n_spec, (uint32_t *)dyn_lds);
}

__global__ __launch_bounds__(256, 8) void k_act_rows(Dev d, int p, int n_active, int n_act_blocks, const uint32_t *__restrict__ bank, int n_inputs,
                                                     int n_rows, int n_duty_blocks) {
    TraceScope ts(d, 0 + 4 * p);
    int b = blockIdx.x;
    if (b < n_act_blocks) {
        const int idx = b * tm_groups_per_block(d) + tm_group_of(d, threadIdx.x);
        const bool ok = idx < n_active;
        const int a = ok ? d.active_cols[p][idx] : 0;
        tm_activate_column(d, p, 1, ok, a, idx, tm_pred_words(d, p, ok, a));
        return;
    }
    b -= n_act_blocks;
    if (b < n_rows) {
        role_sp_row<256>(d, p, bank, n_inputs, 0, b, threadIdx.x);
        return;
    }
    b -= n_rows;
    const int c = b * 256 + (int)threadIdx.x;
    if (b < n_duty_blocks) {
        if (c < d.C) {
            float dc = d.duty[c] * d.mom;
            if ((d.colbits[p][c >> 5] >> (c & 31)) & 1u) dc = dc + d.dinc;
            d.duty[c] = dc;
        }
        return;
    }
    const int n_clear = (int)gridDim.x - n_act_blocks - n_rows - n_duty_blocks;
    for (int w = (b - n_duty_blocks) * 256 + (int)threadIdx.x; w < d.C * d.WPC; w += n_clear * 256) {
        const int cc = w >> (d.LK - 5);
        d.pred[p][w] = 0;
        if (!((d.colbits[p][cc >> 5] >> (cc & 31)) & 1u)) { d.act[p][w] = 0; d.win[p][w] = 0; }
    }
}

__global__ __launch_bounds__(256) void k_mid_overlap(Dev d, int p, int n_active, int want_winner, int learning, int n_cls,
                                                     const uint32_t *__restrict__ bank, int n_inputs, int G, int n_overlap_blocks) {
    TraceScope ts(d, 1 + 4 * p);
    int b = blockIdx.x;
    if (b <= n_cls) {
        role_mid<256>(d, p, n_active, want_winner, learning, b, n_cls);
        return;
    }
    b -= 1 + n_cls;
    if (b < n_overlap_blocks) {
        role_overlap<256>(d, bank, n_inputs, G, p, p ^ 1, 1, b, n_overlap_blocks, (uint32_t *)dyn_lds, 1);
        return;
    }
    b -= n_overlap_blocks;
    const int nz = (int)gridDim.x - 1 - n_cls - n_overlap_blocks;
    const int words4 = ((d.world > 1 ? d.ctr->L : d.ctr->S) + 127) >> 7;
    uint4 *mb = (uint4 *)d.match_bits[p];
    for (int i = b * 256 + (int)threadIdx.x; i < words4; i += nz * 256) mb[i] = make_uint4(0u, 0u, 0u, 0u);
}

__device__ __forceinline__ void fan_signal(const Dev &d, int p, int b) {
    asm volatile("s_waitcnt vmcnt(0)" ::: "memory");
    __syncthreads();
    if (threadIdx.x == 0)
        __hip_atomic_fetch_add(d.fan + (size_t)(p * FAN_COUNTERS + (b & (FAN_COUNTERS - 1))) * FAN_STRIDE, 1u, __ATOMIC_RELAXED, __HIP_MEMORY_SCOPE_AGENT);
}

__device__ __forceinline__ void fan_wait(const Dev &d, int p, uint32_t target) {
    if (threadIdx.x < 64) {
        for (int looks = 0;; ++looks) {
            uint32_t v = threadIdx.x < FAN_COUNTERS
                             ? __hip_atomic_load(d.fan + (size_t)(p * FAN_COUNTERS + (int)threadIdx.x) * FAN_STRIDE, __ATOMIC_RELAXED, __HIP_MEMORY_SCOPE_AGENT) : 0u;
            v = wave_sum(v);
            if (v >= target) break;
            if (looks >= (1 << 18)) {
                if (threadIdx.x == 0) atomicOr(&d.ctr->error, 32);
                break;
            }
#ifndef BITHTM_FAN_SLEEP
#define BITHTM_FAN_SLEEP 4
#endif
            __builtin_amdgcn_s_sleep(BITHTM_FAN_SLEEP);
        }
    }
    __syncthreads();
}

#ifndef BITHTM_LEAN2_WAVES
#define BITHTM_LEAN2_WAVES 8
#endif
__global__ __launch_bounds__(256, BITHTM_LEAN2_WAVES) void k_act_mid_rows(Dev d, int p, int n_active, int n_act_blocks, int learning, int n_cls,
                                                      const uint32_t *__restrict__ bank, int n_inputs, int n_rows, int G, int n_overlap_blocks,
                                                      int n_duty_blocks, int n_clear_blocks, int order) {
    TraceScope ts(d, 0 + 4 * p);
    int b = blockIdx.x;
    int role = 4;
#pragma unroll
    for (int i = 3; i >= 0 && role == 4; --i) {
        const int r = (order >> (4 * i)) & 15;
        const int n = r == 0 ? n_act_blocks : r == 1 ? 1 + n_cls : r == 2 ? n_rows : n_overlap_blocks;
        if (b < n) role = r; else b -= n;
    }
    if (role == 0) {
        const int idx = b * tm_groups_per_block(d) + tm_group_of(d, threadIdx.x);
        const bool ok = idx < n_active;
        const int a = ok ? d.active_cols[p][idx] : 0;
        tm_activate_column<true>(d, p, 1, ok, a, idx, tm_pred_words(d, p, ok, a));
        fan_signal(d, p, b);
        return;
    }
    if (role == 1) {
        role_mid<256>(d, p, n_active, 1, learning, b, n_cls, 1, [&]() { fan_wait(d, p, (uint32_t)n_act_blocks); });
        return;
    }
    if (role == 2) {
        if (n_overlap_blocks > 0) role_sp_row<256, true>(d, p, bank, n_inputs, 0, b, threadIdx.x);
        else role_sp_row<256>(d, p, bank, n_inputs, 0, b, threadIdx.x);
        return;
    }
    if (role == 3) {
        role_overlap<256>(d, bank, n_inputs, G, p, p ^ 1, 1, b, n_overlap_blocks, (uint32_t *)dyn_lds, 1, n_rows > 0 ? 2 : 1);
        return;
    }
    if (b < n_duty_blocks) {
        const int c = b * 256 + (int)threadIdx.x;
        if (c < d.C) {
            float dc = d.duty[c] * d.mom;
            if ((d.colbits[p][c >> 5] >> (c & 31)) & 1u) dc = dc + d.dinc;
            d.duty[c] = dc;
        }
        return;
    }
    b -= n_duty_blocks;
    if (b < n_clear_blocks) {
        for (int w = b * 256 + (int)threadIdx.x; w < d.C * d.WPC; w += n_clear_blocks * 256) {
            const int cc = w >> (d.LK - 5);
            d.pred[p][w] = 0;
            if (!((d.colbits[p][cc >> 5] >> (cc & 31)) & 1u)) { d.act[p][w] = 0; d.win[p][w] = 0; }
        }
        return;
    }
    b -= n_clear_blocks;
    const int nz = (int)gridDim.x - n_act_blocks - 1 - n_cls - n_rows - n_overlap_blocks - n_duty_blocks - n_clear_blocks;
    const int words4 = (d.ctr->S + 127) >> 7;
    uint4 *mb = (uint4 *)d.match_bits[p];
    for (int i = b * 256 + (int)threadIdx.x; i < words4; i += nz * 256) mb[i] = make_uint4(0u, 0u, 0u, 0u);
}

template <int EPL, int MINW, bool TAB = false>
__global__ __launch_bounds__(256, MINW) void k_learn_scan_emit(Dev d, int p, int n_emit_blocks, int n_learn_blocks, int n_scan_blocks, int n_spec) {
    TraceScope ts(d, 2 + 4 * p);
    constexpr bool LARGE = MINW < 6;
    static_assert(!(LARGE && TAB), "the streaming scan reads the cell words from memory");
    const bool dyn = LARGE && n_scan_blocks > 0;
    if (n_scan_blocks < 0) n_scan_blocks = -n_scan_blocks;
    if (blockIdx.x == gridDim.x - 1 && threadIdx.x < FAN_COUNTERS) d.fan[(size_t)(p * FAN_COUNTERS + (int)threadIdx.x) * FAN_STRIDE] = 0u;
    int b = blockIdx.x, scan_blk;
    if (b < n_emit_blocks) {
        role_emit(d, p ^ 1, 1, 1, 0, b, n_emit_blocks, (EmitShared *)dyn_lds, 1);
        if (!dyn) return;
        scan_blk = -1 - b;
    } else if (b < n_emit_blocks + n_learn_blocks) {
        role_learn<EPL, 256, true>(d, p, b - n_emit_blocks, n_learn_blocks, (LearnShared<EPL, 256> *)dyn_lds);
        if (!dyn) return;
        scan_blk = -1 - b;
    } else {
        scan_blk = b - n_emit_blocks - n_learn_blocks;
    }
    if (LARGE) role_scan<256, true, true, false, true>(d, p, scan_blk, n_scan_blocks, dyn ? n_emit_blocks + n_learn_blocks : 0, (uint32_t *)dyn_lds);
    else role_scan<256, true, false, TAB>(d, p, scan_blk, n_scan_blocks, n_spec, (uint32_t *)dyn_lds);
}

template <int EPL>
__global__ __launch_bounds__(256, 6) void k_learn_scan_tail(Dev d, int p, int n_learn_blocks, int n_scan_blocks, int n_spec,
                                                            const uint32_t *__restrict__ bank, int n_inputs, int G, int wmode, int n_rows) {
    int b = blockIdx.x;
    if (blockIdx.x == gridDim.x - 1 && threadIdx.x < FAN_COUNTERS) d.fan[(size_t)(p * FAN_COUNTERS + (int)threadIdx.x) * FAN_STRIDE] = 0u;
    if (b < n_learn_blocks) {
        role_learn<EPL, 256, true>(d, p, b, n_learn_blocks, (LearnShared<EPL, 256> *)dyn_lds);
        return;
    }
    b -= n_learn_blocks;
    if (b < n_scan_blocks) {
        role_scan<256, true, false, false>(d, p, b, n_scan_blocks, n_spec, (uint32_t *)dyn_lds);
        return;
    }
    b -= n_scan_blocks;
    if (n_rows > 0) role_sp_row<256>(d, p, bank, n_inputs, 0, b, threadIdx.x);
    else role_overlap<256>(d, bank, n_inputs, G, p, p ^ 1, 1, b, (int)gridDim.x - n_learn_blocks - n_scan_blocks, (uint32_t *)dyn_lds, wmode);
}

template <int EPL>
__global__ __launch_bounds__(256, 6) void k_learn_scan_front(Dev d, int p_prev, int n_learn_blocks, int n_scan_blocks, int n_spec,
                                                             PackedInputArg in, int G, int p, int wmode) {
    int b = blockIdx.x;
    if (blockIdx.x == gridDim.x - 1 && threadIdx.x < FAN_COUNTERS) d.fan[(size_t)(p_prev * FAN_COUNTERS + (int)threadIdx.x) * FAN_STRIDE] = 0u;
    if (b < n_learn_blocks) {
        role_learn<EPL, 256, true>(d, p_prev, b, n_learn_blocks, (LearnShared<EPL, 256> *)dyn_lds);
        return;
    }
    b -= n_learn_blocks;
    if (b < n_scan_blocks) {
        role_scan<256, true, false, false>(d, p_prev, b, n_scan_blocks, n_spec, (uint32_t *)dyn_lds);
        return;
// ... 14 lines not shown
```

bithtm_amd/csrc/htm_sp_kernels.h:

```cpp
#ifndef BITHTM_HTM_SP_KERNELS_H
#define BITHTM_HTM_SP_KERNELS_H


__global__ __launch_bounds__(256) void k_sp_build_mask(Dev d, int row_begin, int row_count) {
    const int wave = (blockIdx.x * blockDim.x + threadIdx.x) >> 6;
    const int nwaves = (gridDim.x * blockDim.x) >> 6;
    const int lane = lane_id();
    const int chunks = d.Ipad >> 6;
    for (long long t = wave; t < (long long)row_count * chunks; t += nwaves) {
        int row = row_begin + (int)(t / chunks), ch = (int)(t % chunks);
        int i = ch * 64 + lane;
        bool conn = (i < d.I) && (d.perm[(size_t)row * d.Ipad + i] >= d.sp_thr);
        u64 m = __ballot(conn);
        if (lane == 0) *(u64 *)&d.mask[(size_t)row * d.W + ch * 2] = m;
    }
}

#ifdef BITHTM_OVERLAP_STAMPS
#define OV_STAMP(i) do { if (d.trace && wmode && threadIdx.x == 0 && blk < 512) d.trace[(size_t)3 * 8192 + (size_t)blk * 8 + (i)] = wall_clock64(); } while (0)
#else
#define OV_STAMP(i) do { } while (0)
#endif
template <int BS>
__device__ __forceinline__ void role_overlap(const Dev &d, const uint32_t *__restrict__ bank, int n_inputs, int G,
                                             int p, int sp, int step_offset, int blk, int nblk, uint32_t *h, int wmode = 0, int fold = 0) {
    const int gtid = blk * BS + threadIdx.x;
    const int nthreads = nblk * BS;
    uint32_t *ghist = d.hist + sp * SEL_MAX_PASSES * SEL_BINS;
    OV_STAMP(0);
    if (gtid == 0) d.ctr->emit_epoch += 1;
    const uint4 *in4 = (const uint4 *)bank;
    if (n_inputs > 1) in4 = (const uint4 *)(bank + (size_t)((d.ctr->step[p] + (uint32_t)step_offset) % (uint32_t)n_inputs) * d.W);
    const uint4 *mask4 = (const uint4 *)d.mask;
    const int lane = lane_id();
    const int rpw = 64 / G, sub = lane / G, l = lane % G;
    const int wave = gtid >> 6, nwaves = nthreads >> 6;
    constexpr int U = 4;
    const bool spread = G == 8;
    const int first_row0 = d.c0 + wave * rpw * U;
    uint4 m[U];
    float dty_first = 0.f;
    uint32_t cbw_first = 0u;
#pragma unroll
    for (int u = 0; u < U; ++u) {
        const int row = first_row0 + u * rpw + sub;
        m[u] = (row < d.c1 && l < d.W4) ? mask4[(uint32_t)row * (uint32_t)d.W4 + (uint32_t)l] : make_uint4(0, 0, 0, 0);
    }
    if (spread) {
        const int row = first_row0 + (l & 3) * rpw + sub;
        dty_first = (l < U && row < d.c1) ? d.duty[row] : 0.f;
        if (fold) cbw_first = (l < U && row < d.c1) ? d.colbits[p][row >> 5] : 0u;
    }
    for (int i = gtid; i < (d.sel_passes - 1) * SEL_BINS; i += nthreads) ghist[SEL_BINS + i] = 0;
    for (int i = threadIdx.x; i < SEL_BINS; i += BS) h[i] = 0;
    if (gtid == 0) {
        d.ctr->sel_pass_prefix[sp][0] = 0;
        d.ctr->sel_pass_krem[sp][0] = (uint32_t)d.sel_k;
    }
    const uint32_t wbase = wmode ? d.ctr->sel_win[sp] : 0u;
    lds_barrier();
    OV_STAMP(1);
    static_assert(WIN_BINS <= SEL_BINS - SEL_COARSE, "the runs' sums live behind the window's bins in the LDS histogram");
    uint32_t *hc = h + SEL_BINS - SEL_COARSE;
    auto finish_row = [&](bool owner, int row, int cn, float duty, uint32_t cbw) {
        u64 key = 0;
        if (owner && fold) {
            duty = duty * d.mom;
            if ((cbw >> (row & 31)) & 1u) {
                if (fold == 2) owner = false;
                else duty = duty + d.dinc;
            }
            if (owner) d.duty[row] = duty;
        }
        if (owner) {
            d.overlap[sp][row] = cn;
            const float f = htm_exp_f32(d.coef * duty);
            const double bo = (double)f * (double)cn;
            d.boosted[sp][row] = bo;
            key = select_key(bo);
            d.key[sp][row] = key;
        }
        const uint32_t bin = wmode ? win_bin(key, wbase) : (uint32_t)(key >> sel_shift(0));
        if (owner && (!wmode || bin != 0u)) {
            atomicAdd(&h[bin], 1u);
            if (wmode) atomicAdd(&hc[bin >> 6], 1u);
        }
    };
    for (int row0 = first_row0; row0 < d.c1; row0 += nwaves * rpw * U) {
        const bool first = row0 == first_row0;
        int cnt[U];
        float dty = dty_first;
        uint32_t cbw = cbw_first;
#pragma unroll
        for (int u = 0; u < U; ++u) cnt[u] = 0;
        if (!first && spread) {
            const int row = row0 + (l & 3) * rpw + sub;
            dty = (l < U && row < d.c1) ? d.duty[row] : 0.f;
            if (fold) cbw = (l < U && row < d.c1) ? d.colbits[p][row >> 5] : 0u;
        }
        for (int j = l; j < d.W4; j += G) {
            if (!(first && j == l)) {
#pragma unroll
                for (int u = 0; u < U; ++u) {
                    const int row = row0 + u * rpw + sub;
                    m[u] = row < d.c1 ? mask4[(uint32_t)row * (uint32_t)d.W4 + (uint32_t)j] : make_uint4(0, 0, 0, 0);
                }
            }
            const uint4 x = in4[j];
#pragma unroll
            for (int u = 0; u < U; ++u)
                cnt[u] += __popc(m[u].x & x.x) + __popc(m[u].y & x.y) + __popc(m[u].z & x.z) + __popc(m[u].w & x.w);
        }
        OV_STAMP(2);
        if (spread) {
            int mine = 0;
#pragma unroll
            for (int u = 0; u < U; ++u) {
                const int cn = group8_sum_all(cnt[u]);
                if (l == u) mine = cn;
            }
            const int row = row0 + (l & 3) * rpw + sub;
            finish_row(l < U && row < d.c1, row, mine, dty, cbw);
        } else {
#pragma unroll
            for (int u = 0; u < U; ++u) {
                int cn = cnt[u];
                for (int o = G >> 1; o > 0; o >>= 1) cn += __shfl_xor(cn, o);
                const int row = row0 + u * rpw + sub;
                const bool mine = l == 0 && row < d.c1;
                finish_row(mine, row, cn, mine ? d.duty[row] : 0.f, (fold && mine) ? d.colbits[p][row >> 5] : 0u);
            }
        }
    }
    OV_STAMP(3);
    lds_barrier();
    OV_STAMP(4);
    uint32_t *g0 = d.hist0 + (size_t)sp * HIST0_PAR + (size_t)(blk & (HIST_REP - 1)) * SEL_BINS;
    uint32_t *gc = d.hist0 + (size_t)sp * HIST0_PAR + HIST0_FINE + (size_t)(blk & (COARSE_REP - 1)) * COARSE_STRIDE;
    const int n_fine = wmode ? SEL_BINS - SEL_COARSE : SEL_BINS;
    {
        constexpr int PER = SEL_BINS / BS;
        uint32_t v[PER];
#pragma unroll
        for (int k = 0; k < PER; ++k) v[k] = h[threadIdx.x + k * BS];
#pragma unroll
        for (int k = 0; k < PER; ++k) {
            const int i = threadIdx.x + k * BS;
            if (v[k] && i < n_fine) atomicAdd(&g0[i], v[k]);
        }
    }
    if (wmode && threadIdx.x < SEL_COARSE && hc[threadIdx.x]) atomicAdd(&gc[threadIdx.x], hc[threadIdx.x]);
    OV_STAMP(5);
}

__global__ __launch_bounds__(RB) void k_sp_overlap(Dev d, const uint32_t *__restrict__ bank, int n_inputs, int G, int p, int sp, int step_offset, int wmode) {
    __shared__ uint32_t h[SEL_BINS];
    role_overlap<RB>(d, bank, n_inputs, G, p, sp, step_offset, blockIdx.x, gridDim.x, h, wmode);
}

#define ARG_INPUT_WORDS 64
struct PackedInputArg { uint32_t w[ARG_INPUT_WORDS]; };
__global__ __launch_bounds__(RB) void k_sp_overlap_arg(Dev d, PackedInputArg in, int G, int p, int wmode) {
    __shared__ uint32_t h[SEL_BINS];
    __shared__ __attribute__((aligned(16))) uint32_t s_in[ARG_INPUT_WORDS];
    if (threadIdx.x < ARG_INPUT_WORDS) {
        const uint32_t v = threadIdx.x < d.W ? in.w[threadIdx.x] : 0u;
        s_in[threadIdx.x] = v;
        if (blockIdx.x == 0 && threadIdx.x < d.W) d.input_stage[threadIdx.x] = v;
    }
    __syncthreads();
    role_overlap<RB>(d, s_in, 1, G, p, p, 0, blockIdx.x, gridDim.x, h, wmode);
}

template <int BS>
__device__ __forceinline__ void sel_resolve(const Dev &d, int sp, int prev, uint32_t *h, uint32_t *s_wave,
                                            u64 *out_prefix, uint32_t *out_krem, u64 *s_res_prefix, uint32_t *s_res_krem) {
    const int tid = threadIdx.x, lane = lane_id(), wv = tid >> 6;
    const int shift = sel_shift(prev), nb = 1 << sel_bits(prev);
    const u64 prefix = d.ctr->sel_pass_prefix[sp][prev];
    const uint32_t krem = d.ctr->sel_pass_krem[sp][prev];
    const uint32_t *gh = d.hist + (sp * SEL_MAX_PASSES + prev) * SEL_BINS;
    constexpr int PER = SEL_BINS / BS;
    static_assert(PER % 4 == 0, "16-byte histogram accesses");
    {
        uint4 v[PER / 4];
#pragma unroll
        for (int j = 0; j < PER / 4; ++j) {
            const int b = 4 * (j * BS + tid);
            v[j] = (prev > 0 && b < nb) ? *(const uint4 *)(gh + b) : make_uint4(0, 0, 0, 0);
        }
        if (prev == 0) {
            const uint32_t *g0 = d.hist0 + (size_t)sp * HIST0_PAR;
            for (int r = 0; r < HIST_REP; ++r)
#pragma unroll
                for (int j = 0; j < PER / 4; ++j) {
                    const uint4 a = *(const uint4 *)(g0 + (size_t)r * SEL_BINS + 4 * (j * BS + tid));
                    v[j].x += a.x; v[j].y += a.y; v[j].z += a.z; v[j].w += a.w;
                }
        }
#pragma unroll
        for (int j = 0; j < PER / 4; ++j) *(uint4 *)(h + 4 * (j * BS + tid)) = v[j];
    }
    __syncthreads();
    uint32_t cs = 0;
#pragma unroll
    for (int j = 0; j < PER / 4; ++j) {
        const uint4 v = *(const uint4 *)(h + tid * PER + 4 * j);
        cs += v.x + v.y + v.z + v.w;
    }
    const uint32_t pre = wave_incl_scan(cs);
    const uint32_t wtot = (uint32_t)__builtin_amdgcn_readlane((int)pre, 63);
    if (lane == 0) s_wave[wv] = wtot;
    __syncthreads();
    uint32_t above = wtot - pre;
    for (int w = wv + 1; w < BS / 64; ++w) above += s_wave[w];
    if (above < krem && krem <= above + cs) {
        for (int b = min((tid + 1) * PER, nb) - 1; b >= tid * PER; --b) {
            const uint32_t hb = h[b];
            if (above + hb >= krem) {
                *s_res_prefix = prefix | ((u64)b << shift);
                *s_res_krem = krem - above;
                break;
            }
            above += hb;
        }
    }
    __syncthreads();
    *out_prefix = *s_res_prefix;
    *out_krem = *s_res_krem;
}

struct SelShared { uint32_t h[SEL_BINS]; uint32_t wave[16]; u64 prefix; uint32_t krem; };

template <int BS>
__device__ __forceinline__ void role_sel_pass(const Dev &d, int pass, int sp, int blk, int nblk, SelShared *sh) {
// ... 843 lines not shown
            atomicAdd(&s_n, 1);
        }
        if (d.act[0] && (mode & EMIT_CLEAR)) {
            for (int h = 0; h < d.WPC; ++h) {
                d.pred[p][c * d.WPC + h] = 0;
                if (!sel || !(mode & EMIT_ACTIVATE)) { d.act[p][c * d.WPC + h] = 0; d.win[p][c * d.WPC + h] = 0; }
            }
        }
    }
    if (b == 0 && tid == 0 && !d.act[0]) d.ctr->step[p ^ 1] = d.ctr->step[p] + 1;
    EMIT_STAMP(5);
    if (!tm_here && !local) return;
    __syncthreads();
    const int n_sel = s_n;
    if (local) {
        double *r_boost = (double *)d.send;
        uint32_t *r_col = (uint32_t *)(d.send + (size_t)d.cand_cap * 8), *r_win = r_col + d.cand_cap, *r_unacc = r_win + d.cand_cap;
        const int has_distal = d.ctr->has_distal;
        const uint32_t step = d.ctr->step[p];
        constexpr int CPP = 4;
        for (int i0 = 0; i0 < n_sel; i0 += 8 * CPP) {
            int a[CPP];
            bool ok[CPP];
            ColumnLoads l[CPP];
            double bo[CPP];
#pragma unroll
            for (int u = 0; u < CPP; ++u) {
                const int i = i0 + u * 8 + (tid >> 5);
                ok[u] = i < n_sel;
                a[u] = ok[u] ? s_col[i] : d.c0;
                l[u] = tm_column_loads(d, p, ok[u], a[u], has_distal);
                bo[u] = d.boosted[p][a[u]];
            }
#pragma unroll
            for (int u = 0; u < CPP; ++u) {
                const ColumnWords w = tm_column_compute(d, 1, ok[u], a[u], ok[u] ? s_predw[a[u] - cbase] : 0u, l[u], has_distal, step);
                const int pos = first_pos + i0 + u * 8 + (tid >> 5);
                if (ok[u] && (lane & 31) == 0) {
                    r_boost[pos] = bo[u];
                    r_col[pos] = (uint32_t)a[u] | (w.burst ? 0x80000000u : 0u);
                    r_win[pos] = w.winner;
                    r_unacc[pos] = w.unacc;
                }
            }
        }
        for (int i = d.sel_k + b * 256 + tid; i < d.cand_cap; i += nblk * 256) ((u64 *)r_boost)[i] = CAND_PAD;
        if (b == 0) {
            uint32_t *r_dead = r_unacc + d.cand_cap;
            const int n = min(d.dead_list[0], DEAD_CAP);
            if (tid == 0) {
                r_dead[0] = (uint32_t)n;
                uint32_t *r_n = (uint32_t *)(d.send + shard_record_count_offset(d.cand_cap));
                r_n[0] = (uint32_t)d.sel_k;
                r_n[1] = CAND_HOT_NONE;
                if (fused && wmode) d.ctr->cand_exact += 1;
            }
            for (int j = tid; j < n; j += 256) r_dead[1 + j] = (uint32_t)d.dead_list[1 + j];
        }
        return;
    }
    for (int i0 = 0; i0 < n_sel; i0 += tm_groups_per_block(d)) {
        const int i = i0 + tm_group_of(d, tid);
        const bool ok = i < n_sel;
        const int a = ok ? s_col[i] : 0;
        tm_activate_column(d, p, want_winner, ok, a, first_pos + i, d.WPC == 1 ? (u64)(ok ? s_predw[a - cbase] : 0u) : tm_pred_words(d, p, ok, a));
    }
}

__global__ __launch_bounds__(256) void k_sp_emit(Dev d, int p, int want_winner, int fused, int mode, int wmode, int n_emit_blocks) {
    __shared__ EmitShared sh;
    if ((int)blockIdx.x >= n_emit_blocks) {
        const int nb = (int)gridDim.x - n_emit_blocks;
        for (int c = ((int)blockIdx.x - n_emit_blocks) * 256 + (int)threadIdx.x; c < d.C * d.WPC; c += nb * 256) {
            d.act[p][c] = 0;
            d.win[p][c] = 0;
            d.pred[p][c] = 0;
            if (c < d.colwords) d.colbits[p][c] = 0;
        }
        return;
    }
    role_emit(d, p, want_winner, fused, mode, blockIdx.x, n_emit_blocks, &sh, wmode);
}

__device__ __forceinline__ void role_sp_learn_row(const Dev &d, const uint32_t *__restrict__ bank, int n_inputs, int p, int b) {
    const uint32_t *in = bank + (size_t)(d.ctr->step[p] % (uint32_t)n_inputs) * d.W;
    const int row = d.active_cols[p][b];
    double *prow = d.perm + (size_t)row * d.Ipad;
    uint32_t *mrow = d.mask + (size_t)row * d.W;
    for (int i0 = 0; i0 < d.Ipad; i0 += 256) {
        int i = i0 + threadIdx.x;
        bool conn = false;
        if (i < d.I) {
            bool on = (in[i >> 5] >> (i & 31)) & 1u;
            double v = prow[i] + (on ? d.sp_don : d.sp_doff);
            prow[i] = v;
            conn = v >= d.sp_thr;
        }
        u64 m = __ballot(conn);
        if (lane_id() == 0 && i < d.Ipad) *(u64 *)&mrow[i >> 5] = m;
    }
}

__global__ __launch_bounds__(256) void k_sp_learn(Dev d, const uint32_t *__restrict__ bank, int n_inputs, int p) {
    role_sp_learn_row(d, bank, n_inputs, p, (int)blockIdx.x);
}

enum { SP_KEYS_HOST = 0, SP_KEYS_BOOST = 1 };
__global__ __launch_bounds__(RB) void k_sp_keys(Dev d, int p, int from_overlap) {
    __shared__ uint32_t h[SEL_BINS];
    const int gtid = blockIdx.x * RB + threadIdx.x, nthreads = gridDim.x * RB;
    uint32_t *ghist = d.hist + p * SEL_MAX_PASSES * SEL_BINS;
    if (gtid == 0) {
        d.ctr->emit_epoch += 1;
        d.ctr->sel_pass_prefix[p][0] = 0;
        d.ctr->sel_pass_krem[p][0] = (uint32_t)d.sel_k;
    }
    for (int i = gtid; i < (d.sel_passes - 1) * SEL_BINS; i += nthreads) ghist[SEL_BINS + i] = 0;
    for (int i = threadIdx.x; i < SEL_BINS; i += RB) h[i] = 0;
    __syncthreads();
    for (int c = d.sel_lo + gtid; c < d.sel_hi; c += nthreads) {
        double bo;
        if (from_overlap) {
            const float f = htm_exp_f32(d.coef * d.duty[c]);
            bo = (double)f * (double)d.overlap[p][c];
            d.boosted[p][c] = bo;
        } else {
            bo = d.boosted[p][c];
        }
        const u64 key = from_overlap ? select_key(bo) : (u64)__double_as_longlong(bo) & 0x7FFFFFFFFFFFFFFFull;
        d.key[p][c] = key;
        atomicAdd(&h[(uint32_t)(key >> sel_shift(0))], 1u);
    }
    __syncthreads();
    uint32_t *g0 = d.hist0 + (size_t)p * HIST0_PAR + (size_t)(blockIdx.x & (HIST_REP - 1)) * SEL_BINS;
    for (int i = threadIdx.x; i < SEL_BINS; i += RB)
        if (h[i]) atomicAdd(&g0[i], h[i]);
}

__global__ __launch_bounds__(256) void k_sp_list_bits(Dev d, int p, int n, int pass) {
    const int i = blockIdx.x * 256 + threadIdx.x;
    if (pass == 0) { if (i < d.colwords) d.colbits[p][i] = 0; return; }
    if (i < n) { const int c = d.active_cols[p][i]; atomicOr(&d.colbits[p][c >> 5], 1u << (c & 31)); }
}

__global__ __launch_bounds__(256) void k_sp_duty_list(Dev d, int p, int n, int pass) {
    const int i = blockIdx.x * 256 + threadIdx.x;
    if (pass == 0) { if (i < d.C) d.duty[i] = d.duty[i] * d.mom; return; }
    if (i < n) { const int c = d.active_cols[p][i]; d.duty[c] = d.duty[c] + d.dinc; }
}

__global__ void k_sp_commit(Dev d, int p) { d.ctr->step[p ^ 1] = d.ctr->step[p] + 1; }

__global__ __launch_bounds__(RB) void k_shard_overlap(Dev d, const uint32_t *__restrict__ bank, int n_inputs, int G, int p, int wmode, int front) {
    __shared__ uint32_t h[SEL_BINS];
    role_overlap<RB>(d, bank, n_inputs, G, p, front ? p ^ 1 : p, front ? 1 : 0, blockIdx.x, gridDim.x, h, wmode);
}

struct BlockSelLds { uint32_t *h, *s_wave, *s_out, *s_cnt; u64 *s_or, *s_and; unsigned long long *trace; };
#ifdef BITHTM_SHARD_STAMPS
#define SHARD_STAMP(i) do { if (d.trace && blockIdx.x == 0 && threadIdx.x == 0) d.trace[i] = wall_clock64(); } while (0)
#define SEL_STAMP(i) do { if (L.trace && blockIdx.x == 0 && threadIdx.x == 0) L.trace[i] = wall_clock64(); } while (0)
#else
#define SHARD_STAMP(i) do { } while (0)
#define SEL_STAMP(i) do { } while (0)
#endif

template <int KPT>
__device__ __forceinline__ void block_select_regs(const u64 (&kreg)[KPT], uint32_t vmask, uint32_t k, uint32_t base, int low_zero,
                                                  const BlockSelLds &L, u64 *T_out, uint32_t *r_out, bool *missed, bool h_zeroed = false) {
    const int tid = threadIdx.x, lane = lane_id();
    uint32_t *h = L.h;
    u64 P = 0;
    uint32_t krem = k;
    bool done = false;
    u64 T = 0;
    int top_start = 64, top0 = 64;
    bool outside = false;
    {
        if (!h_zeroed) {
            for (int i = tid; i < SEL_BINS; i += 1024) h[i] = 0;
            if (tid == 0) { L.s_cnt[0] = 0; L.s_out[0] = 0; *L.s_or = 0; *L.s_and = ~0ull; }
// ... 398 lines not shown
```

bithtm_amd/csrc/htm_sp_run.h:

```cpp

struct SpRecDev {
    int32_t *cols;
    int32_t *overlap;
    double *boosted;
    uint32_t base;
    int32_t n;
};

__global__ void k_sp_run_begin(SpRecDev *r, int32_t *cols, int32_t *overlap, double *boosted, uint32_t base, int32_t n) {
    if (blockIdx.x == 0 && threadIdx.x == 0) {
        r->cols = cols;
        r->overlap = overlap;
        r->boosted = boosted;
        r->base = base;
        r->n = n;
    }
}

__global__ __launch_bounds__(256) void k_sp_run_tail(Dev d, const uint32_t *__restrict__ bank, int n_inputs, int p, int n_learn, const SpRecDev *__restrict__ r) {
    const int b = (int)blockIdx.x;
    if (b < n_learn) {
        role_sp_learn_row(d, bank, n_inputs, p, b);
        return;
    }
    const int i = (b - n_learn) * 256 + (int)threadIdx.x;
    const uint32_t slot = d.ctr->step[p] - r->base;
    if (i >= d.k || slot >= (uint32_t)r->n) return;
    const int col = d.active_cols[p][i];
    const size_t at = (size_t)slot * d.k + i;
    if (r->cols) r->cols[at] = col;
    if (r->overlap) r->overlap[at] = d.overlap[p][col];
    if (r->boosted) r->boosted[at] = d.boosted[p][col];
}
```

bithtm_amd/csrc/htm_tm_kernels.h:

```cpp
#ifndef BITHTM_HTM_TM_KERNELS_H
#define BITHTM_HTM_TM_KERNELS_H


__global__ __launch_bounds__(256) void k_tm_load_active(Dev d, int p, const int *cols, int n) {
    for (int c = blockIdx.x * 256 + threadIdx.x; c < d.C * d.WPC; c += gridDim.x * 256) {
        d.act[p][c] = 0;
        d.pred[p][c] = 0;
        d.win[p][c] = 0;
        if (c < n) d.active_cols[p][c] = cols[c];
        if (c < d.colwords) d.colbits[p][c] = 0;
    }
}

__global__ __launch_bounds__(256) void k_tm_activate(Dev d, int p, int n_active, int want_winner) {
    const int idx = blockIdx.x * tm_groups_per_block(d) + tm_group_of(d, threadIdx.x);
    const bool ok = idx < n_active;
    const int a = ok ? d.active_cols[p][idx] : 0;
    if (ok && (threadIdx.x & (d.KP - 1)) == 0) atomicOr(&d.colbits[p][a >> 5], 1u << (a & 31));
    tm_activate_column(d, p, want_winner, ok, a, idx, tm_pred_words(d, p, ok, a));
}

__global__ __launch_bounds__(256) void k_tm_ext_winners(Dev d, int p, const int *cols, const uint32_t *winw, const uint32_t *unacc, int n, int pass) {
    const int i = blockIdx.x * 256 + threadIdx.x;
    if (pass == 0) { for (int c = i; c < d.C * d.WPC; c += gridDim.x * 256) d.win[p][c] = 0; return; }
// ... 31 lines not shown
        const int n = min(*count, d.work_cap);
        for (int i = blockIdx.x * 256 + threadIdx.x; i < n; i += gridDim.x * 256) d.work[i] = list[i] | 0x80000000u;
        if (blockIdx.x == 0 && threadIdx.x == 0) { c->n_work[p] = n; c->n_bind[p] = 0; }
        return;
    }
    if (!c->has_distal) return;
    const int q = p ^ 1, n = c->S;
    for (int base = blockIdx.x * 256; base < n; base += gridDim.x * 256) {
        const int seg = base + (int)threadIdx.x;
        bool pun = false;
        if (seg < n && ((d.match_bits[q][seg >> 5] >> (seg & 31)) & 1u)) {
            const int cell = d.seg_cell[seg];
            pun = (punish[cell >> 5] >> (cell & 31)) & 1u;
        }
        const u64 m = __ballot(pun);
        if (!m) continue;
        int b = 0;
        if (lane_id() == 0) b = atomicAdd(count, __popcll(m));
        b = wave_read(b, 0);
        if (pun) {
            const int pos = b + __popcll(m & lanemask_lt());
            if (pos < d.work_cap) list[pos] = (uint32_t)seg; else atomicOr(&c->error, 4);
        }
    }
}

__device__ __forceinline__ bool col_is_local(const Dev &d, int cell) { const int col = cell >> d.LK; return col >= d.c0 && col < d.c1; }

__device__ __forceinline__ int seg_gid_of(const Dev &d, int row) { return d.seg_gid ? d.seg_gid[row] : row; }

__device__ __forceinline__ void tm_bind_segment(const Dev &d, int seg, int cell, bool recycled, int pos) {
    if (recycled) atomicSub(&d.segcount[d.seg_cell[seg]], 1);
    d.seg_cell[seg] = cell;
    d.seg_nsyn[seg] = (int)SEG_BUSY;
    atomicAdd(&d.segcount[cell], 1);
    if (pos < d.work_cap) d.work[pos] = (uint32_t)seg; else atomicOr(&d.ctr->error, 4);
}

__device__ __forceinline__ void shard_bind(const Dev &d, int p, int gid, int cell, bool recycled, int grown, int pass) {
    Counters *c = d.ctr;
    const bool to_me = col_is_local(d, cell);
    const int old_row = recycled ? d.g2l[gid] : -1;
    if (pass == 0) {
        const bool alive = grown >= d.match_thr;
        if (recycled && alive) { atomicAnd(&d.dead_bits[gid >> 5], ~(1u << (gid & 31))); recyc_add(d, gid >> 10, -1); }
        if (!recycled && !alive) { atomicOr(&d.dead_bits[gid >> 5], 1u << (gid & 31)); recyc_add(d, gid >> 10, 1); }
        if (old_row >= 0) {
            atomicSub(&d.segcount[d.seg_cell[old_row]], 1);
            if (!to_me) {
                d.seg_gid[old_row] = -1;
                d.seg_nsyn[old_row] = 0;
                d.g2l[gid] = -1;
                d.lfree[atomicAdd(&c->n_lfree, 1)] = old_row;
            }
        }
        return;
    }
    if (!to_me) return;
    int row = old_row;
    if (row < 0) {
        const int top = atomicSub(&c->n_lfree, 1) - 1;
        if (top >= 0) {
            row = d.lfree[top];
        } else {
            atomicAdd(&c->n_lfree, 1);
            row = atomicAdd(&c->L, 1);
        }
        if (row >= d.Lcap) { atomicOr(&c->error, 1); return; }
        d.seg_gid[row] = gid;
        d.g2l[gid] = row;
    }
    d.seg_cell[row] = cell;
    d.seg_nsyn[row] = (int)SEG_BUSY;
    atomicAdd(&d.segcount[cell], 1);
    const int pos = atomicAdd(&c->n_work[p], 1);
    if (pos < d.work_cap) d.work[pos] = (uint32_t)row; else atomicOr(&c->error, 4);
}

#ifdef BITHTM_ROWS_STAMPS
#define ROW_STAMP(i) do { if (d.trace && t == 0 && ri < 1024) d.trace[(size_t)7 * 8192 + (size_t)ri * 8 + (i)] = wall_clock64(); } while (0)
#else
#define ROW_STAMP(i) do { } while (0)
#endif
template <int TPR, bool OWN = false>
__device__ __forceinline__ void role_sp_row(const Dev &d, int p, const uint32_t *__restrict__ bank, int n_inputs, int ahead, int ri, int t) {
    ROW_STAMP(0);
    const uint32_t step = ahead ? d.ctr->step[p ^ 1] + 1u : d.ctr->step[p];
    const uint32_t *in = bank + (size_t)(step % (uint32_t)n_inputs) * d.W;
    const uint32_t *in_next = bank + (size_t)((step + 1u) % (uint32_t)n_inputs) * d.W;
    const int row = d.active_cols[p][ri];
    if (row < d.c0 || row >= d.c1) return;
    ROW_STAMP(1);
    double *prow = d.perm + (size_t)row * d.Ipad;
    uint32_t *mrow = d.mask + (size_t)row * d.W;
    float duty0 = 0.f;
    uint32_t wbase = 0u;
    if (OWN && t == 0) {
        duty0 = d.duty[row];
        wbase = d.ctr->sel_win[p ^ 1];
    }
    int own_cn = 0;
    for (int i0 = 0; i0 < d.Ipad; i0 += 2 * TPR) {
        const int e0 = i0 + 2 * t;
        bool c0 = false, c1 = false;
        if (e0 < d.Ipad) {
            double2 v = *(double2 *)(prow + e0);
            const uint32_t bits = in[e0 >> 5] >> (e0 & 31);
            const uint32_t nbits = OWN ? in_next[e0 >> 5] >> (e0 & 31) : 0u;
            if (e0 < d.I) { v.x = v.x + ((bits & 1u) ? d.sp_don : d.sp_doff); c0 = v.x >= d.sp_thr; }
            if (e0 + 1 < d.I) { v.y = v.y + ((bits & 2u) ? d.sp_don : d.sp_doff); c1 = v.y >= d.sp_thr; }
            if (OWN) own_cn += (int)(c0 && (nbits & 1u)) + (int)(c1 && (nbits & 2u));
            if (i0 == 0) ROW_STAMP(2); else ROW_STAMP(4);
            {
                typedef unsigned int u32x4 __attribute__((ext_vector_type(4)));
                union { double2 d2; u32x4 u4; } cvt;
                cvt.d2 = v;
                double *dst = prow + e0;
                asm volatile("global_store_dwordx4 %0, %1, off sc0 sc1\n\ts_nop 1" ::"v"(dst), "v"(cvt.u4) : "memory");
            }
        }
        const u64 b0 = __ballot(c0), b1 = __ballot(c1);
        const int base = i0 + 2 * (t & ~63);
        if (lane_id() == 0 && base < d.Ipad) {
            u64 *mw = (u64 *)&mrow[base >> 5];
            const u64 m0 = spread32((uint32_t)b0) | (spread32((uint32_t)b1) << 1);
            const u64 m1 = spread32((uint32_t)(b0 >> 32)) | (spread32((uint32_t)(b1 >> 32)) << 1);
            mw[0] = m0;
            mw[1] = m1;
        }
        if (i0 == 0) ROW_STAMP(3); else ROW_STAMP(5);
    }
    if (OWN) {
        __shared__ int s_own[TPR / 64];
        own_cn = (int)wave_sum((uint32_t)own_cn);
        if (lane_id() == 0) s_own[t >> 6] = own_cn;
        __syncthreads();
        if (t == 0) {
            int cn = 0;
#pragma unroll
            for (int wv = 0; wv < TPR / 64; ++wv) cn += s_own[wv];
            const int sp = p ^ 1;
            float dc = duty0 * d.mom;
            dc = dc + d.dinc;
            d.duty[row] = dc;
            d.overlap[sp][row] = cn;
            const float f = htm_exp_f32(d.coef * dc);
            const double bo = (double)f * (double)cn;
            d.boosted[sp][row] = bo;
            const u64 key = select_key(bo);
            d.key[sp][row] = key;
            const uint32_t bin = win_bin(key, wbase);
            if (bin != 0u) {
                atomicAdd(d.hist0 + (size_t)sp * HIST0_PAR + (size_t)(ri & (HIST_REP - 1)) * SEL_BINS + bin, 1u);
                atomicAdd(d.hist0 + (size_t)sp * HIST0_PAR + HIST0_FINE + (size_t)(ri & (COARSE_REP - 1)) * COARSE_STRIDE + (bin >> 6), 1u);
            }
        }
    }
}

template <typename T>
__device__ __forceinline__ T ld_agent(const T *ptr, int same_launch) {
    return same_launch ? __hip_atomic_load(ptr, __ATOMIC_RELAXED, __HIP_MEMORY_SCOPE_AGENT) : *ptr;
}
struct NoWait { __device__ __forceinline__ void operator()() const {} };
template <int BS, typename Wait = NoWait>
__device__ __forceinline__ void role_mid(const Dev &d, int p, int n_active, int want_winner, int learning, int blk, int n_cls, int same_launch = 0,
                                         Wait wait = Wait()) {
    Counters *c = d.ctr;
    __shared__ int s_words[BS];
    __shared__ uint32_t s_bits[BS];
    __shared__ int s_nwords;
    if (blk > 0) {
        if (!learning || !c->has_distal) return;
        const int q = p ^ 1;
        const int n = d.world > 1 ? c->L : c->S;
        bool waited = false;
        auto wait_once = [&]() { if (!waited) { wait(); waited = true; } };
        auto gather = [&](int seg, bool &cand, bool &punish, int &cell) {
            const uint32_t info = d.seg_info[seg];
            cell = d.seg_cell[seg];
            const float jit = d.seg_jit[seg];
            const int cw = cell >> 5, cb = cell & 31, col = cell >> d.LK;
            const bool on_col = (d.colbits[p][col >> 5] >> (col & 31)) & 1u;
            const bool unpred = !((d.pred[q][cw] >> cb) & 1u);
            const bool best = fabsf(jit - __uint_as_float(d.cellmax[q][cell])) < d.eps;
            cand = ((info >> 31) || (unpred && best)) && (on_col || !same_launch);
            punish = d.punish ? (d.punish[cw] >> cb) & 1u : !on_col;
        };
        auto decide = [&](bool cand, int cell) {
            return cand && ((ld_agent(&d.win[p][cell >> 5], same_launch) >> (cell & 31)) & 1u);
        };
        if (n <= (d.cls_rows_max >= 0 ? d.cls_rows_max : (same_launch ? 2 : 8) * n_cls * BS)) {
            for (int i0 = (blk - 1) * BS; i0 < n; i0 += n_cls * BS) {
                const int seg = i0 + (int)threadIdx.x;
                bool cand = false, punish = false;
                int cell = 0;
                if (seg < n && ((d.match_bits[q][seg >> 5] >> (seg & 31)) & 1u)) gather(seg, cand, punish, cell);
                wait_once();
                const bool learn = decide(cand, cell);
                if (learn || punish) d.seg_nsyn[seg] |= (int)SEG_BUSY;
                const u64 ml = __ballot(learn), mp = __ballot(punish);
                const int n_l = __popcll(ml), n_p = __popcll(mp);
                if (n_l + n_p == 0) continue;
                int base = 0;
                if (lane_id() == 0) base = atomicAdd(&c->n_work[p], n_l + n_p);
                base = wave_read(base, 0);
                if (learn) {
                    const int pos = base + __popcll(ml & lanemask_lt());
                    if (pos < d.work_cap) d.work[pos] = (uint32_t)seg; else atomicOr(&c->error, 4);
                }
                if (punish) {
// ... 1123 lines not shown
```

bithtm_amd/engine.py:

```python

import contextlib
import ctypes as C

import numpy as np

from . import _lib as L


class HtmError(RuntimeError):
    pass


class CapacityError(HtmError):
    """The fixed-capacity segment pool or a segment's synapse slots are exhausted."""


def pack_bits(bits, words):
    if type(bits) is np.ndarray and bits.dtype == np.uint32 and bits.ndim == 1 and bits.size == words and bits.flags.c_contiguous:
        return bits
    bits = np.asarray(bits)
    if bits.dtype != np.bool_:
        bits = bits.astype(np.bool_)
    packed = np.packbits(bits, bitorder="little")
    if packed.size == words * 4:
# ... 140 lines not shown

    def carry_from(self, old):
        self._auto_grow = old._auto_grow

    @classmethod
    def view_of(cls, parent):
        v = cls.__new__(cls)
        for a in cls._VIEW_ATTRS:
            if a in parent.__dict__:
                setattr(v, a, parent.__dict__[a])
        handle = C.c_void_p()
        rc = v.lib.htm_create_view(parent.h, C.byref(handle))
        if rc != 0:
            raise HtmError(f"htm_create_view failed ({rc}): {v.lib.htm_last_error(None).decode()}")
        v.h = handle
        v._host_state(auto_grow=False, stream_owner=parent._stream_owner)
        v.is_view = True
        return v

    def view_sync(self, source):
        self._check(self.lib.htm_view_sync(self.h, source.h), "htm_view_sync")
        self.steps = source.steps

    def bank_rows(self, device_bank, bank_rows, first_step, n, device_dst):
        self._check(self.lib.htm_bank_rows(self.h, C.c_void_p(device_bank), int(bank_rows), int(first_step), int(n), C.c_void_p(device_dst)),
                    "htm_bank_rows")

    def device_bytes(self):
        return int(self._check(self.lib.htm_device_bytes(self.h), "htm_device_bytes"))

    def __del__(self):
        h, self.h = getattr(self, "h", None), None
        if h:
            self.lib.htm_destroy(h)
        for ptr, _ in getattr(self, "_record_bufs", {}).values():
            self.lib.hipFree(ptr)
        for ptr in list(getattr(self, "_reset_bufs", {}).values()) + list(getattr(self, "_list_bufs", {}).values()):
            self.lib.hipFree(ptr)
        for pair in getattr(self, "_value_bufs", {}).values():
            for ptr in pair:
                self.lib.hipFree(ptr)

    def _check(self, rc, what):
        if rc < 0:
            raise HtmError(f"{what} failed ({rc}): {self.lib.htm_last_error(self.h).decode()}")
        return rc

    def info(self):
        out = L.HtmInfo()
        rc = self.lib.htm_get_info(self.h, C.byref(out))
        if rc != -3:
            self._check(rc, "htm_get_info")
        return out

    def check_capacity(self):
        info = self.info()
        if info.capacity_error:
            raise CapacityError(self.lib.htm_last_error(self.h).decode())
        return info

    def pool_look(self, per_step, force=False):
        if not self._auto_grow or not self.has_tm:
            return False
        every = self.POOL_LOOK_EVERY
        self._since_check += 1
        if self._since_check < every and not force:
            return False
        self._since_check = 0
        info = self.check_capacity()
        self._free_segments = self.segment_capacity - info.segments
        capacity = slots = None
        if self._free_segments < (every + 1) * per_step:
            capacity = max(2 * self.segment_capacity, info.segments + 4 * (every + 1) * per_step)
        if info.segments and self.segment_slots < 512:
            nsyn = self.read(L.F_SEG_NSYN, np.int32, info.local_segments)
            if int(nsyn.max(initial=0)) > 3 * self.segment_slots // 4:
                slots = min(512, 2 * self.segment_slots)
        self._grow_to = (capacity, slots)
        return capacity is not None or slots is not None

    def sync(self):
        self._check(self.lib.htm_sync(self.h), "htm_sync")

    def stream_handle(self):
        out = C.c_void_p()
        self._check(self.lib.htm_get_stream(self.h, C.byref(out)), "htm_get_stream")
        return out.value or 0

    def shard_run(self, device_bank, n_inputs, n_steps, learning=True, use_graph=True, pipeline=True):
        self._check(self.lib.htm_shard_run(self.h, C.c_void_p(device_bank), int(n_inputs), int(n_steps), int(bool(learning)),
                                           run_flags(use_graph, pipeline)), "htm_shard_run")
        self.steps += n_steps

    def import_prev_state(self, prediction, activation, winner_flat, distal):
        K = self.cell_dim
        S = self.info().segments
        self._check(self.lib.htm_import_begin(self.h, -1), "htm_import_begin")
        self.write(L.F_CELL_PREDICTION, bool_to_words(np.asarray(prediction).reshape(self.column_dim, K)), np.uint32)
        self.write(L.F_CELL_ACTIVATION, bool_to_words(np.asarray(activation).reshape(self.column_dim, K)), np.uint32)
        winners = np.zeros(0, np.int32) if winner_flat is None else np.asarray(winner_flat, dtype=np.int32)
        self.write(L.F_WINNER_CELL, winners, np.int32)
        M = 0
        if distal is not None:
            seg = np.asarray(distal.matching_segment, dtype=np.int32)
            M = len(seg)
            pot = np.zeros(S, dtype=np.int64)
            old = np.asarray(distal.segment_potential, dtype=np.int64)[:S]
            pot[:len(old)] = old
            minfo = (pot[seg].astype(np.uint32) | (np.asarray(distal.matching_segment_activation).astype(np.uint32) << 12)
                     | (np.asarray(distal.matching_segment_active).astype(np.uint32) << 31))
            self.write(L.F_SEG_POTENTIAL, pot, np.int32)
            self.write(L.F_MATCH_SEGMENT, seg, np.int32)
            self.write(L.F_MATCH_INFO, minfo, np.uint32)
            self.write(L.F_MATCH_JITTER, np.asarray(distal.matching_segment_jittered_potential, dtype=np.float32), np.float32)
            self.write(L.F_CELL_MAX_JITTER, np.asarray(distal.max_jittered_potential, dtype=np.float32).view(np.uint32), np.uint32)
        self._check(self.lib.htm_import_commit(self.h, int(S), int(M), len(winners), int(distal is not None), int(winner_flat is not None)),
                    "htm_import_commit")

    def reset(self):
        self._check(self.lib.htm_reset(self.h), "htm_reset")

    def upload_resets(self, resets):
        bits = np.ascontiguousarray(np.asarray(resets, dtype=np.bool_).ravel())
        key = (bits.size, bits.tobytes())
        bufs = self._reset_bufs
        if key not in bufs:
            words = np.zeros((bits.size + 31) // 32 * 4, dtype=np.uint8)
            pb = np.packbits(bits, bitorder="little")
            words[:pb.size] = pb
            bufs[key] = self.device_buffer(words.size, words)
        return bufs[key]

    def set_run_resets(self, device_bits, n_inputs):
        self._check(self.lib.htm_set_run_resets(self.h, C.c_void_p(device_bits) if device_bits else None, int(n_inputs)),
                    "htm_set_run_resets")

    def set_epsilon(self, epsilon):
        self._check(self.lib.htm_set_epsilon(self.h, C.c_float(float(epsilon))), "htm_set_epsilon")

    def use_epsilon(self, epsilon):
        if self._epsilon != epsilon:
            self.set_epsilon(epsilon)
            self._epsilon = epsilon

    def this_call(self, resets=None, n_inputs=0, feedback=None, votes=None):
        if resets is None and feedback is None and votes is None:
            return _NOTHING_TO_SET
        return self._settings(resets, n_inputs, feedback, votes)

    @contextlib.contextmanager
    def _settings(self, resets, n_inputs, feedback, votes):
        undo = []
        try:
            if resets is not None:
                self.set_run_resets(resets, n_inputs)
                undo.append(lambda: self.set_run_resets(None, 0))
            if feedback is not None:
                self.set_run_feedback(*feedback)
                undo.append(lambda: self.set_run_feedback(None))
            if votes is not None:
                self.set_run_predicted_input(votes)
                undo.append(lambda: self.set_run_predicted_input(None))
            yield
        finally:
            for clear in reversed(undo):
                clear()
# ... 514 lines not shown
```

include/bithtm_hip.h:

```cpp
#ifndef BITHTM_HIP_H
#define BITHTM_HIP_H

#include <stddef.h>
#include <stdint.h>

#ifdef __cplusplus
extern "C" {
#endif

#define BITHTM_ABI_VERSION 4

typedef struct htm_handle htm_handle;

typedef enum htm_status {
    HTM_OK = 0,
    HTM_ERR_ARGUMENT = -1,
    HTM_ERR_HIP = -2,
    HTM_ERR_CAPACITY = -3,
    HTM_ERR_STATE = -4
} htm_status;

typedef struct htm_config {
    uint32_t struct_bytes;
    int32_t device;
// ... 4 lines not shown
    int32_t enable_sp;
    int32_t enable_tm;
    double sp_permanence_threshold;
    double sp_delta_on;
    double sp_delta_off;
    float boost_coefficient;
    float duty_momentum;
    float duty_increment;
    double tm_learn_active;
    double tm_learn_inactive;
    double tm_punish_active;
    double tm_punish_inactive;
    int32_t tm_learn_prune;
    int32_t tm_punish_prune;
    float tm_permanence_initial;
    float tm_permanence_threshold;
    int32_t segment_activation_threshold;
    int32_t segment_matching_threshold;
    int32_t segment_sampling_synapses;
    int32_t segment_capacity;
    int32_t segment_capacity_local;
    int32_t segment_slots;
    uint32_t seed;
    int32_t shard_rank;
    int32_t shard_world;
    int32_t use_caller_stream;
    void *stream;
} htm_config;

typedef struct htm_info {
    int64_t step_index;
    int32_t segments;
    int32_t local_segments;
    int32_t matching_segments;
    int32_t winner_cells;
    int32_t active_cells;
    int32_t has_distal_state;
    int32_t has_winner_cells;
    int32_t capacity_error;
    int32_t words_per_row;
    int32_t new_segment_requests;
    int32_t recycled_segments;
    int32_t appended_segments;
    int32_t work_items;
    int32_t select_fallbacks;
    int32_t candidate_exact_steps;
    int32_t hot_select_steps;
    int32_t select_zoom_steps;
} htm_info;

typedef enum htm_field {
    HTM_F_ACTIVE_COLUMN = 1,
    HTM_F_OVERLAPS = 2,
    HTM_F_BOOSTED = 3,
    HTM_F_DUTY_CYCLE = 4,
    HTM_F_CELL_ACTIVATION = 5,
    HTM_F_CELL_PREDICTION = 6,
    HTM_F_WINNER_WORDS = 7,
    HTM_F_BURSTING = 8,
    HTM_F_WINNER_CELL = 9,
    HTM_F_SEG_CELL = 10,
    HTM_F_SEG_NSYN = 11,
    HTM_F_SEG_PRESYN = 12,
    HTM_F_SEG_PERM = 13,
    HTM_F_SEGCOUNT = 14,
    HTM_F_SEG_POTENTIAL = 15,
    HTM_F_MATCH_SEGMENT = 16,
    HTM_F_MATCH_INFO = 17,
    HTM_F_MATCH_JITTER = 18,
    HTM_F_CELL_MAX_JITTER = 19,
    HTM_F_SEG_GID = 20,
    HTM_F_RECYCLABLE_COUNTS = 21
} htm_field;

int htm_create(const htm_config *config, htm_handle **out);
void htm_destroy(htm_handle *h);
const char *htm_last_error(const htm_handle *h);
int htm_abi_version(void);

int htm_sp_set_permanence(htm_handle *h, const double *rows, int32_t row_begin, int32_t row_count);

int htm_set_epsilon(htm_handle *h, float epsilon);
int htm_sp_get_permanence(htm_handle *h, double *rows, int32_t row_begin, int32_t row_count);

int htm_step(htm_handle *h, const uint32_t *packed_input, int32_t learning);
int htm_sp_step(htm_handle *h, const uint32_t *packed_input, int32_t learning);
int htm_tm_step(htm_handle *h, const int32_t *active_column, int32_t n, int32_t learning,
                int32_t return_winner_cell);

int htm_tm_update(htm_handle *h, const int32_t *columns, const uint32_t *winner_words, const uint32_t *unaccounted_words,
                  int32_t n, const uint32_t *punish_words);
int htm_tm_scan(htm_handle *h, const uint32_t *active_words);

typedef enum htm_sp_phase_id {
    HTM_SP_OVERLAP = 1,
    HTM_SP_BOOST = 2,
    HTM_SP_SELECT = 3,
    HTM_SP_ACTIVE = 4,
    HTM_SP_LEARN = 5,
    HTM_SP_DUTY = 6,
    HTM_SP_COMMIT = 7
} htm_sp_phase_id;
int htm_sp_phase(htm_handle *h, int32_t phase, const void *data, int64_t count);

int htm_run(htm_handle *h, const uint32_t *device_inputs, int32_t n_inputs, int32_t n_steps,
            int32_t learning, int32_t use_graph);
#define HTM_RUN_GRAPH 1
#define HTM_RUN_NO_PIPELINE 2
#define HTM_RUN_CONTINUE 4

int htm_prepare(htm_handle *h, const uint32_t *device_inputs, int32_t n_inputs, int32_t n_steps,
                int32_t learning, int32_t use_graph);

#define HTM_PLAN_GRAPH 1
#define HTM_PLAN_PIPELINED 2
#define HTM_PLAN_LEAN 4
#define HTM_PLAN_SCAN_LARGE 8
int htm_run_plan(htm_handle *h, int32_t n_steps, int32_t use_graph);

typedef struct htm_step_record {
    int32_t active_columns;
    int32_t bursting_columns;
    int32_t predicted_columns_before;
    int32_t predicted_columns;
    int32_t active_cells;
    int32_t winner_cells;
    int32_t segments;
    int32_t new_segments;
} htm_step_record;

typedef struct htm_run_record {
    uint32_t struct_bytes;
    htm_step_record *records;
    int32_t *active_column;
    uint32_t *column_prediction;
} htm_run_record;

int htm_run_recorded(htm_handle *h, const uint32_t *device_inputs, int32_t n_inputs, int32_t n_steps, int32_t learning,
                     int32_t use_graph, const htm_run_record *rec);
int htm_prepare_recorded(htm_handle *h, const uint32_t *device_inputs, int32_t n_inputs, int32_t n_steps, int32_t learning,
                         int32_t use_graph);
int htm_reset(htm_handle *h);
int htm_set_run_resets(htm_handle *h, const uint32_t *device_bits, int32_t n_inputs);
int htm_predicted_input(htm_handle *h, int32_t *host_dst);
int htm_set_run_predicted_input(htm_handle *h, int32_t *device_votes);

int htm_graph_count(htm_handle *h);

int htm_bank_upload(htm_handle *h, const uint32_t *host_inputs, int32_t n_inputs, uint32_t **device_bank);

int64_t htm_shard_record_bytes(htm_handle *h);
int htm_shard_begin(htm_handle *h, const uint32_t *device_inputs, int32_t n_inputs, const uint32_t *packed_input,
                    int32_t learning, void *send_device);
int htm_shard_finish(htm_handle *h, const void *recv_device, int32_t learning);

int htm_shard_unique_id(void *out128);
int htm_shard_comm_init(htm_handle *h, const void *unique_id128);
int htm_shard_step(htm_handle *h, const uint32_t *device_inputs, int32_t n_inputs, const uint32_t *packed_input,
                   int32_t learning);
int htm_shard_comm_size(htm_handle *h);
int htm_shard_graph_ok(htm_handle *h);
int htm_shard_run(htm_handle *h, const uint32_t *device_inputs, int32_t n_inputs, int32_t n_steps, int32_t learning, int32_t use_graph);
int htm_shard_group_run(htm_handle *const *handles, int32_t n, const uint32_t *const *device_inputs, int32_t n_inputs, int32_t n_steps,
                        int32_t learning, int32_t use_graph);
int htm_rccl_selftest(int32_t device);

// ... 112 lines not shown
```

Baseline: 42210 timesteps/s.

## Add transposed byte-plane mask layout for sparse-input SP overlap

Keeps a column-major byte-plane copy of the SP connection mask (one plane per input byte, columns contiguous) and computes overlap by walking only the non-zero input bytes, with each thread counting four columns via coalesced plane reads. The plane copy is kept in sync by diff-stores in the SP learning paths. This is meant to cut the overlap cost from scanning every mask word of every column to touching only the planes for active input bytes. In exchange it adds extra memory, extra scattered byte stores during learning, and a check kernel for consistency.

Result: faster. 42840 timesteps/s, median of 6 (+1.5%).

```diff
diff --git a/bithtm_amd/_lib.py b/bithtm_amd/_lib.py
--- a/bithtm_amd/_lib.py
+++ b/bithtm_amd/_lib.py
@@ -117,6 +117,7 @@
     "htm_shard_group_step": (C.c_int, [C.POINTER(C.c_void_p), C.c_int32, C.POINTER(C.c_void_p), C.c_int32, C.c_void_p, C.c_int32]),
     "htm_populate": (C.c_int, [C.c_void_p, C.c_int64, C.c_int64, C.c_int32, C.c_int32, C.c_double, C.c_double, C.c_uint32]),
     "htm_sync": (C.c_int, [C.c_void_p]),
+    "htm_sp_planes_check": (C.c_int, [C.c_void_p, C.POINTER(C.c_int64)]),
     "htm_get_stream": (C.c_int, [C.c_void_p, C.POINTER(C.c_void_p)]),
     "htm_get_info": (C.c_int, [C.c_void_p, C.POINTER(HtmInfo)]),
     "htm_read": (C.c_int64, [C.c_void_p, C.c_int32, C.c_void_p, C.c_int64]),
diff --git a/bithtm_amd/csrc/htm_dev.h b/bithtm_amd/csrc/htm_dev.h
--- a/bithtm_amd/csrc/htm_dev.h
+++ b/bithtm_amd/csrc/htm_dev.h
@@ -78,6 +78,7 @@
     uint32_t sel_win_global;
     u64 sel_pass_prefix[2][SEL_MAX_PASSES + 1];
     uint32_t sel_pass_krem[2][SEL_MAX_PASSES + 1];
+    uint32_t plane_steps;
 };
 
 struct Dev {
@@ -149,6 +150,8 @@
     Counters *ctr;
     unsigned long long *trace;
     uint32_t trace_until;
+    int plane_stride;
+    uint8_t *planes;
 };
 
 __device__ __forceinline__ int lane_id() { return threadIdx.x & 63; }
diff --git a/bithtm_amd/csrc/htm_engine.hip b/bithtm_amd/csrc/htm_engine.hip
--- a/bithtm_amd/csrc/htm_engine.hip
+++ b/bithtm_amd/csrc/htm_engine.hip
@@ -59,6 +59,7 @@
     int G;
     int sp_blocks, sel_blocks, c256_blocks, s1024_blocks, scan_blocks, zero_blocks, cus;
     int lean_learn_blocks, lean_learn_blocks_large, lean_scan_blocks, lean_scan_blocks_large, lean_overlap_blocks, lean2_classify_blocks;
+    int lean2_overlap_blocks;
     int lean_resident_large;
     bool emit_fits, emit_fits_open;
     bool emit_fits_lean;
@@ -163,6 +164,7 @@
     long long seen_wgen;
     uint32_t dense_step;
     int64_t own_bytes;
+    unsigned long long *d_planes_bad;
 };
 
 struct HtmShared {
@@ -456,9 +458,10 @@
     const int n_cls = learning ? kClassifyBlocks : 0, n_ov = plan.next_sp ? h->sz.lean_overlap_blocks : 0;
     if (h->knob.lean == 2) {
         const int n_cls2 = lean2_classify_blocks(h, learning);
-        const int n_duty = n_ov ? 0 : h->sz.c256_blocks, n_clear = d.WPC * h->sz.c256_blocks;
+        const int n_ov2 = plan.next_sp ? h->sz.lean2_overlap_blocks : 0;
+        const int n_duty = n_ov2 ? 0 : h->sz.c256_blocks, n_clear = d.WPC * h->sz.c256_blocks;
         LAUNCH_ON(h, h->stream, (size_t)SEL_BINS * 4, "tm_activate+tm_mid+sp_learn+sp_overlap", k_act_mid_rows,
-                  n_act + 1 + n_cls2 + n_rows + n_ov + n_duty + n_clear + h->sz.zero_blocks, 256, d, p, d.k, n_act, learning, n_cls2, bank, n_inputs, n_rows, h->sz.G, n_ov,
+                  n_act + 1 + n_cls2 + n_rows + n_ov2 + n_duty + n_clear + h->sz.zero_blocks, 256, d, p, d.k, n_act, learning, n_cls2, bank, n_inputs, n_rows, h->sz.G, n_ov2,
                   n_duty, n_clear, h->knob.lean2_order);
     } else {
         LAUNCH(h, "tm_activate+sp_learn", k_act_rows, n_act + n_rows + (1 + d.WPC) * h->sz.c256_blocks, 256, d, p, d.k, n_act, bank, n_inputs, n_rows, h->sz.c256_blocks);
@@ -610,6 +613,8 @@
     if (cfg->enable_sp) {
         rc |= dalloc_weights(h, &d.perm, C * d.Ipad);
         rc |= dalloc_weights(h, &d.mask, C * d.W);
+        d.plane_stride = (d.C + 255) & ~255;
+        if (h->world == 1 && C * d.W < ((size_t)1 << 32)) rc |= dalloc_weights(h, &d.planes, (size_t)4 * d.W * d.plane_stride);
     }
     if (cfg->enable_tm) {
         const size_t S = d.Lcap, E = d.E, KP = d.KP;
@@ -766,6 +771,7 @@
     if (z.scan_blocks > 256) z.scan_blocks = (z.scan_blocks + 255) & ~255;
     z.zero_blocks = std::max(1, std::min((d.Lcap / 128 + 4095) / 4096, 1024));
     z.lean_overlap_blocks = k.lean_overlap ? k.lean_overlap : z.sp_blocks * (RB / 256);
+    z.lean2_overlap_blocks = d.planes ? (d.c1 - d.c0 + 255) / 256 : z.lean_overlap_blocks;
     z.lean_learn_blocks = k.lean_learn ? k.lean_learn : 512;
     z.lean_learn_blocks_large = k.lean_learn_large ? k.lean_learn_large : k.lean_learn ? z.lean_learn_blocks : 768;
     z.lean_scan_blocks = k.lean_scan ? k.lean_scan : (z.scan_blocks > 512 ? std::max(256, (z.scan_blocks * 3 / 8 + 255) & ~255) : z.scan_blocks);
@@ -1209,6 +1215,7 @@
     const long long waves = (long long)row_count * (d.Ipad / 64);
     const int blocks = (int)std::min<long long>((waves + 3) / 4, 8192);
     hipLaunchKernelGGL(k_sp_build_mask, dim3(blocks), dim3(256), 0, h->stream, d, row_begin, row_count);
+    if (d.planes) hipLaunchKernelGGL(k_sp_build_planes, dim3((row_count + 63) / 64, (4 * d.W + 63) / 64), dim3(256), 0, h->stream, d, row_begin, row_count);
     HIPCHK(h, hipStreamSynchronize(h->stream));
     return HTM_OK;
 }
@@ -1224,6 +1231,29 @@
     HIPCHK(h, hipMemcpy2DAsync(rows, (size_t)d.I * 8, d.perm + (size_t)row_begin * d.Ipad, (size_t)d.Ipad * 8,
                                (size_t)d.I * 8, (size_t)row_count, hipMemcpyDeviceToHost, h->stream));
     HIPCHK(h, hipStreamSynchronize(h->stream));
+    return HTM_OK;
+}
+
+extern "C" int htm_sp_planes_check(htm_handle *h, int64_t out[2]) {
+    if (!h || !out) return HTM_ERR_ARGUMENT;
+    flush_tail(h);
+    if (!h->cfg.enable_sp) { h->err = "handle has no Spatial Pooler"; return HTM_ERR_STATE; }
+    Dev &d = h->d;
+    HIPCHK(h, hipSetDevice(h->device));
+    uint32_t steps = 0;
+    HIPCHK(h, hipStreamSynchronize(h->stream));
+    HIPCHK(h, hipMemcpy(&steps, &d.ctr->plane_steps, sizeof(steps), hipMemcpyDeviceToHost));
+    out[0] = -1;
+    out[1] = (int64_t)steps;
+    if (!d.planes) return HTM_OK;
+    if (!h->d_planes_bad) { if (int rc = dalloc(h, &h->d_planes_bad, 1)) return rc; }
+    HIPCHK(h, hipMemsetAsync(h->d_planes_bad, 0, sizeof(unsigned long long), h->stream));
+    const size_t total = (size_t)4 * d.W * d.plane_stride;
+    hipLaunchKernelGGL(k_sp_planes_check, dim3((unsigned)std::min<size_t>((total + 255) / 256, 4096)), dim3(256), 0, h->stream, d, h->d_planes_bad);
+    unsigned long long bad = 0;
+    HIPCHK(h, hipMemcpyAsync(&bad, h->d_planes_bad, sizeof(bad), hipMemcpyDeviceToHost, h->stream));
+    HIPCHK(h, hipStreamSynchronize(h->stream));
+    out[0] = (int64_t)bad;
     return HTM_OK;
 }
 
diff --git a/bithtm_amd/csrc/htm_pipeline.h b/bithtm_amd/csrc/htm_pipeline.h
--- a/bithtm_amd/csrc/htm_pipeline.h
+++ b/bithtm_amd/csrc/htm_pipeline.h
@@ -105,7 +105,7 @@
     }
     b -= n_act_blocks;
     if (b < n_rows) {
-        role_sp_row<256>(d, p, bank, n_inputs, 0, b, threadIdx.x);
+        role_sp_row<256, false, false>(d, p, bank, n_inputs, 0, b, threadIdx.x);
         return;
     }
     b -= n_rows;
@@ -206,7 +206,8 @@
         return;
     }
     if (role == 3) {
-        role_overlap<256>(d, bank, n_inputs, G, p, p ^ 1, 1, b, n_overlap_blocks, (uint32_t *)dyn_lds, 1, n_rows > 0 ? 2 : 1);
+        if (d.planes) role_overlap_planes(d, bank, n_inputs, p, p ^ 1, 1, b, n_overlap_blocks, (uint32_t *)dyn_lds, n_rows > 0 ? 2 : 1);
+        else role_overlap<256>(d, bank, n_inputs, G, p, p ^ 1, 1, b, n_overlap_blocks, (uint32_t *)dyn_lds, 1, n_rows > 0 ? 2 : 1);
         return;
     }
     if (b < n_duty_blocks) {
diff --git a/bithtm_amd/csrc/htm_sp_kernels.h b/bithtm_amd/csrc/htm_sp_kernels.h
--- a/bithtm_amd/csrc/htm_sp_kernels.h
+++ b/bithtm_amd/csrc/htm_sp_kernels.h
@@ -16,11 +16,110 @@
     }
 }
 
+__global__ __launch_bounds__(256) void k_sp_build_planes(Dev d, int row_begin, int row_count) {
+    __shared__ uint8_t tile[64][68];
+    const int c0 = row_begin + (int)blockIdx.x * 64, c_end = row_begin + row_count;
+    const int w0 = (int)blockIdx.y * 16;
+    for (int i = threadIdx.x; i < 64 * 16; i += 256) {
+        const int c = c0 + (i >> 4), w = w0 + (i & 15);
+        const uint32_t v = (c < c_end && w < d.W) ? d.mask[(size_t)c * d.W + w] : 0u;
+        *(uint32_t *)&tile[i >> 4][(i & 15) * 4] = v;
+    }
+    __syncthreads();
+    for (int i = threadIdx.x; i < 64 * 64; i += 256) {
+        const int c = c0 + (i & 63), j = w0 * 4 + (i >> 6);
+        if (c < c_end && j < 4 * d.W) d.planes[(size_t)j * d.plane_stride + c] = tile[i & 63][i >> 6];
+    }
+}
+
+__global__ __launch_bounds__(256) void k_sp_planes_check(Dev d, unsigned long long *bad) {
+    unsigned long long n = 0;
+    const size_t total = (size_t)4 * d.W * d.plane_stride;
+    for (size_t i = (size_t)blockIdx.x * 256 + threadIdx.x; i < total; i += (size_t)gridDim.x * 256) {
+        const int j = (int)(i / d.plane_stride), c = (int)(i % d.plane_stride);
+        const uint8_t want = c < d.C ? ((const uint8_t *)(d.mask + (size_t)c * d.W))[j] : (uint8_t)0;
+        n += d.planes[i] != want;
+    }
+    n = wave_reduce64(n, 0ull, [](u64 a, u64 b) { return a + b; });
+    if (lane_id() == 0 && n) atomicAdd(bad, n);
+}
+
+__device__ __forceinline__ uint32_t plane_old_byte(const Dev &d, const uint32_t *mrow, int byte0) {
+    return ((const uint8_t *)mrow)[min(byte0 + (lane_id() & 15), 4 * d.W - 1)];
+}
+template <int NB>
+__device__ __forceinline__ void plane_diff_store(const Dev &d, int row, int byte0, bool valid, u64 m0, u64 m1, uint32_t old) {
+    const int j = lane_id();
+    const uint32_t nb = (uint32_t)(((j & 8) ? m1 : m0) >> (8 * (j & 7))) & 0xFFu;
+    if (d.planes && valid && j < NB && nb != old) d.planes[(size_t)(byte0 + j) * d.plane_stride + row] = (uint8_t)nb;
+}
+template <int NB, bool ROW_FROM_MROW = false>
+__device__ __forceinline__ void plane_diff_store_late(const Dev &d, const uint32_t *mrow, int row, int i0, u64 m0, u64 m1) {
+    if (!d.planes) return;
+    int t = (int)threadIdx.x;
+    asm volatile("" : "+v"(t));
+    const int j = t & 63, byte0 = (i0 >> 3) + NB * (t >> 6);
+    if (byte0 * 8 < d.Ipad && j < NB) {
+        const uint32_t old = ((const uint8_t *)mrow)[byte0 + j];
+        const uint32_t nb = (uint32_t)(((j & 8) ? m1 : m0) >> (8 * (j & 7))) & 0xFFu;
+        if (nb != old) {
+            if (ROW_FROM_MROW) row = (int)((uint32_t)(mrow - d.mask) / (uint32_t)d.W);
+            d.planes[(size_t)(byte0 + j) * d.plane_stride + row] = (uint8_t)nb;
+        }
+    }
+}
+
 #ifdef BITHTM_OVERLAP_STAMPS
 #define OV_STAMP(i) do { if (d.trace && wmode && threadIdx.x == 0 && blk < 512) d.trace[(size_t)3 * 8192 + (size_t)blk * 8 + (i)] = wall_clock64(); } while (0)
 #else
 #define OV_STAMP(i) do { } while (0)
 #endif
+__device__ __forceinline__ void overlap_finish_row(const Dev &d, int sp, int wmode, int fold, uint32_t wbase, uint32_t *h, uint32_t *hc,
+                                                   bool owner, int row, int cn, float duty, uint32_t cbw) {
+    u64 key = 0;
+    if (owner && fold) {
+        duty = duty * d.mom;
+        if ((cbw >> (row & 31)) & 1u) {
+            if (fold == 2) owner = false;
+            else duty = duty + d.dinc;
+        }
+        if (owner) d.duty[row] = duty;
+    }
+    if (owner) {
+        d.overlap[sp][row] = cn;
+        const float f = htm_exp_f32(d.coef * duty);
+        const double bo = (double)f * (double)cn;
+        d.boosted[sp][row] = bo;
+        key = select_key(bo);
+        d.key[sp][row] = key;
+    }
+    const uint32_t bin = wmode ? win_bin(key, wbase) : (uint32_t)(key >> sel_shift(0));
+    if (owner && (!wmode || bin != 0u)) {
+        atomicAdd(&h[bin], 1u);
+        if (wmode) atomicAdd(&hc[bin >> 6], 1u);
+    }
+}
+
+template <int BS>
+__device__ __forceinline__ void overlap_flush_hist(const Dev &d, int sp, int blk, int wmode, const uint32_t *h) {
+    const uint32_t *hc = h + SEL_BINS - SEL_COARSE;
+    uint32_t *g0 = d.hist0 + (size_t)sp * HIST0_PAR + (size_t)(blk & (HIST_REP - 1)) * SEL_BINS;
+    uint32_t *gc = d.hist0 + (size_t)sp * HIST0_PAR + HIST0_FINE + (size_t)(blk & (COARSE_REP - 1)) * COARSE_STRIDE;
+    const int n_fine = wmode ? SEL_BINS - SEL_COARSE : SEL_BINS;
+    {
+        constexpr int PER = SEL_BINS / BS;
+        uint32_t v[PER];
+#pragma unroll
+        for (int k = 0; k < PER; ++k) v[k] = h[threadIdx.x + k * BS];
+#pragma unroll
+        for (int k = 0; k < PER; ++k) {
+            const int i = threadIdx.x + k * BS;
+            if (v[k] && i < n_fine) atomicAdd(&g0[i], v[k]);
+        }
+    }
+    if (wmode && threadIdx.x < SEL_COARSE && hc[threadIdx.x]) atomicAdd(&gc[threadIdx.x], hc[threadIdx.x]);
+}
+
 template <int BS>
 __device__ __forceinline__ void role_overlap(const Dev &d, const uint32_t *__restrict__ bank, int n_inputs, int G,
                                              int p, int sp, int step_offset, int blk, int nblk, uint32_t *h, int wmode = 0, int fold = 0) {
@@ -63,28 +162,7 @@
     static_assert(WIN_BINS <= SEL_BINS - SEL_COARSE, "the runs' sums live behind the window's bins in the LDS histogram");
     uint32_t *hc = h + SEL_BINS - SEL_COARSE;
     auto finish_row = [&](bool owner, int row, int cn, float duty, uint32_t cbw) {
-        u64 key = 0;
-        if (owner && fold) {
-            duty = duty * d.mom;
-            if ((cbw >> (row & 31)) & 1u) {
-                if (fold == 2) owner = false;
-                else duty = duty + d.dinc;
-            }
-            if (owner) d.duty[row] = duty;
-        }
-        if (owner) {
-            d.overlap[sp][row] = cn;
-            const float f = htm_exp_f32(d.coef * duty);
-            const double bo = (double)f * (double)cn;
-            d.boosted[sp][row] = bo;
-            key = select_key(bo);
-            d.key[sp][row] = key;
-        }
-        const uint32_t bin = wmode ? win_bin(key, wbase) : (uint32_t)(key >> sel_shift(0));
-        if (owner && (!wmode || bin != 0u)) {
-            atomicAdd(&h[bin], 1u);
-            if (wmode) atomicAdd(&hc[bin >> 6], 1u);
-        }
+        overlap_finish_row(d, sp, wmode, fold, wbase, h, hc, owner, row, cn, duty, cbw);
     };
     for (int row0 = first_row0; row0 < d.c1; row0 += nwaves * rpw * U) {
         const bool first = row0 == first_row0;
@@ -151,6 +229,77 @@
     }
     if (wmode && threadIdx.x < SEL_COARSE && hc[threadIdx.x]) atomicAdd(&gc[threadIdx.x], hc[threadIdx.x]);
     OV_STAMP(5);
+}
+
+__device__ __forceinline__ void role_overlap_planes(const Dev &d, const uint32_t *__restrict__ bank, int n_inputs, int p, int sp, int step_offset,
+                                                    int blk, int nblk, uint32_t *h, int fold) {
+    constexpr int BS = 256, PB = 8;
+    const int t = threadIdx.x, lane = lane_id(), wv = t >> 6;
+    const int gtid = blk * BS + t, nthreads = nblk * BS;
+    uint32_t *ghist = d.hist + sp * SEL_MAX_PASSES * SEL_BINS;
+    const int row = d.c0 + blk * BS + t;
+    const bool owner = row < d.c1;
+    const int rowc = owner ? row : d.c1 - 1;
+    const float dty = d.duty[rowc];
+    const uint32_t cbw = fold ? d.colbits[p][rowc >> 5] : 0u;
+    if (gtid == 0) {
+        d.ctr->emit_epoch += 1;
+        d.ctr->plane_steps += 1;
+        d.ctr->sel_pass_prefix[sp][0] = 0;
+        d.ctr->sel_pass_krem[sp][0] = (uint32_t)d.sel_k;
+    }
+    for (int i = gtid; i < (d.sel_passes - 1) * SEL_BINS; i += nthreads) ghist[SEL_BINS + i] = 0;
+    const uint32_t wbase = d.ctr->sel_win[sp];
+    const uint32_t *in = bank;
+    if (n_inputs > 1) in = bank + (size_t)((d.ctr->step[p] + (uint32_t)step_offset) % (uint32_t)n_inputs) * d.W;
+    uint32_t *list = h, *s_n = h + 256;
+    uint32_t *s_cnt = h + 512;
+    const uint8_t *pl = d.planes + (size_t)(d.c0 + blk * BS + 4 * lane);
+    int cnt[4] = {0, 0, 0, 0};
+    for (int b0 = 0; b0 < 4 * d.W; b0 += BS) {
+        const int bi = b0 + t;
+        const uint32_t byte = bi < 4 * d.W ? (in[bi >> 2] >> (8 * (bi & 3))) & 0xFFu : 0u;
+        const u64 live = __ballot(byte != 0u);
+        if (lane == 0) s_n[wv] = (uint32_t)__popcll(live);
+        lds_barrier();
+        uint32_t pos = (uint32_t)__popcll(live & lanemask_lt()), n = 0;
+#pragma unroll
+        for (int w = 0; w < BS / 64; ++w) {
+            const uint32_t nw = s_n[w];
+            if (w < wv) pos += nw;
+            n += nw;
+        }
+        if (byte != 0u) list[pos] = (uint32_t)bi | (byte << 16);
+        lds_barrier();
+        for (uint32_t e0 = (uint32_t)wv; e0 < n; e0 += (BS / 64) * PB) {
+            uint32_t ent[PB], word[PB];
+#pragma unroll
+            for (int u = 0; u < PB; ++u) {
+                const uint32_t e = e0 + (uint32_t)u * (BS / 64);
+                ent[u] = e < n ? list[e] : 0u;
+            }
+#pragma unroll
+            for (int u = 0; u < PB; ++u) word[u] = *(const uint32_t *)(pl + (size_t)(ent[u] & 0xFFFFu) * d.plane_stride);
+#pragma unroll
+            for (int u = 0; u < PB; ++u) {
+                const uint32_t v = ent[u] >> 16;
+#pragma unroll
+                for (int i = 0; i < 4; ++i) cnt[i] += __popc(word[u] & (v << (8 * i)));
+            }
+        }
+        lds_barrier();
+    }
+    *(uint4 *)&s_cnt[(wv * 64 + lane) * 4] = make_uint4((uint32_t)cnt[0], (uint32_t)cnt[1], (uint32_t)cnt[2], (uint32_t)cnt[3]);
+    lds_barrier();
+    int cn = 0;
+#pragma unroll
+    for (int w = 0; w < BS / 64; ++w) cn += (int)s_cnt[(w * 64 + (t >> 2)) * 4 + (t & 3)];
+    lds_barrier();
+    for (int i = t; i < SEL_BINS; i += BS) h[i] = 0;
+    lds_barrier();
+    overlap_finish_row(d, sp, 1, fold, wbase, h, h + SEL_BINS - SEL_COARSE, owner, row, cn, dty, cbw);
+    lds_barrier();
+    overlap_flush_hist<BS>(d, sp, blk, 1, h);
 }
 
 __global__ __launch_bounds__(RB) void k_sp_overlap(Dev d, const uint32_t *__restrict__ bank, int n_inputs, int G, int p, int sp, int step_offset, int wmode) {
@@ -1160,6 +1309,7 @@
     role_emit(d, p, want_winner, fused, mode, blockIdx.x, n_emit_blocks, &sh, wmode);
 }
 
+template <bool ROW_FROM_MROW = false>
 __device__ __forceinline__ void role_sp_learn_row(const Dev &d, const uint32_t *__restrict__ bank, int n_inputs, int p, int b) {
     const uint32_t *in = bank + (size_t)(d.ctr->step[p] % (uint32_t)n_inputs) * d.W;
     const int row = d.active_cols[p][b];
@@ -1175,6 +1325,7 @@
             conn = v >= d.sp_thr;
         }
         u64 m = __ballot(conn);
+        plane_diff_store_late<8, ROW_FROM_MROW>(d, mrow, ROW_FROM_MROW ? 0 : row, i0, m, 0ull);
         if (lane_id() == 0 && i < d.Ipad) *(u64 *)&mrow[i >> 5] = m;
     }
 }
diff --git a/bithtm_amd/csrc/htm_sp_run.h b/bithtm_amd/csrc/htm_sp_run.h
--- a/bithtm_amd/csrc/htm_sp_run.h
+++ b/bithtm_amd/csrc/htm_sp_run.h
@@ -20,7 +20,7 @@
 __global__ __launch_bounds__(256) void k_sp_run_tail(Dev d, const uint32_t *__restrict__ bank, int n_inputs, int p, int n_learn, const SpRecDev *__restrict__ r) {
     const int b = (int)blockIdx.x;
     if (b < n_learn) {
-        role_sp_learn_row(d, bank, n_inputs, p, b);
+        role_sp_learn_row<true>(d, bank, n_inputs, p, b);
         return;
     }
     const int i = (b - n_learn) * 256 + (int)threadIdx.x;
diff --git a/bithtm_amd/csrc/htm_tm_kernels.h b/bithtm_amd/csrc/htm_tm_kernels.h
--- a/bithtm_amd/csrc/htm_tm_kernels.h
+++ b/bithtm_amd/csrc/htm_tm_kernels.h
@@ -137,7 +137,7 @@
 #else
 #define ROW_STAMP(i) do { } while (0)
 #endif
-template <int TPR, bool OWN = false>
+template <int TPR, bool OWN = false, bool PLANES = true>
 __device__ __forceinline__ void role_sp_row(const Dev &d, int p, const uint32_t *__restrict__ bank, int n_inputs, int ahead, int ri, int t) {
     ROW_STAMP(0);
     const uint32_t step = ahead ? d.ctr->step[p ^ 1] + 1u : d.ctr->step[p];
@@ -158,7 +158,10 @@
     for (int i0 = 0; i0 < d.Ipad; i0 += 2 * TPR) {
         const int e0 = i0 + 2 * t;
         bool c0 = false, c1 = false;
+        const int base = i0 + 2 * (t & ~63);
+        uint32_t old = 0u;
         if (e0 < d.Ipad) {
+            if (PLANES) old = plane_old_byte(d, mrow, base >> 3);
             double2 v = *(double2 *)(prow + e0);
             const uint32_t bits = in[e0 >> 5] >> (e0 & 31);
             const uint32_t nbits = OWN ? in_next[e0 >> 5] >> (e0 & 31) : 0u;
@@ -171,17 +174,29 @@
                 union { double2 d2; u32x4 u4; } cvt;
                 cvt.d2 = v;
                 double *dst = prow + e0;
+                if (PLANES) asm volatile("" : "+v"(old));
                 asm volatile("global_store_dwordx4 %0, %1, off sc0 sc1\n\ts_nop 1" ::"v"(dst), "v"(cvt.u4) : "memory");
             }
         }
         const u64 b0 = __ballot(c0), b1 = __ballot(c1);
-        const int base = i0 + 2 * (t & ~63);
-        if (lane_id() == 0 && base < d.Ipad) {
-            u64 *mw = (u64 *)&mrow[base >> 5];
+        if (PLANES) {
             const u64 m0 = spread32((uint32_t)b0) | (spread32((uint32_t)b1) << 1);
             const u64 m1 = spread32((uint32_t)(b0 >> 32)) | (spread32((uint32_t)(b1 >> 32)) << 1);
-            mw[0] = m0;
-            mw[1] = m1;
+            if (lane_id() == 0 && base < d.Ipad) {
+                u64 *mw = (u64 *)&mrow[base >> 5];
+                mw[0] = m0;
+                mw[1] = m1;
+            }
+            plane_diff_store<16>(d, row, base >> 3, base < d.Ipad, m0, m1, old);
+        } else {
+            const u64 m0 = spread32((uint32_t)b0) | (spread32((uint32_t)b1) << 1);
+            const u64 m1 = spread32((uint32_t)(b0 >> 32)) | (spread32((uint32_t)(b1 >> 32)) << 1);
+            plane_diff_store_late<16>(d, mrow, row, i0, m0, m1);
+            if (lane_id() == 0 && base < d.Ipad) {
+                u64 *mw = (u64 *)&mrow[base >> 5];
+                mw[0] = m0;
+                mw[1] = m1;
+            }
         }
         if (i0 == 0) ROW_STAMP(3); else ROW_STAMP(5);
     }
diff --git a/bithtm_amd/engine.py b/bithtm_amd/engine.py
--- a/bithtm_amd/engine.py
+++ b/bithtm_amd/engine.py
@@ -246,6 +246,11 @@
     def sync(self):
         self._check(self.lib.htm_sync(self.h), "htm_sync")
 
+    def planes_check(self):
+        out = (C.c_int64 * 2)()
+        self._check(self.lib.htm_sp_planes_check(self.h, out), "htm_sp_planes_check")
+        return int(out[0]), int(out[1])
+
     def stream_handle(self):
         out = C.c_void_p()
         self._check(self.lib.htm_get_stream(self.h, C.byref(out)), "htm_get_stream")
diff --git a/include/bithtm_hip.h b/include/bithtm_hip.h
--- a/include/bithtm_hip.h
+++ b/include/bithtm_hip.h
@@ -110,6 +110,7 @@
 
 int htm_set_epsilon(htm_handle *h, float epsilon);
 int htm_sp_get_permanence(htm_handle *h, double *rows, int32_t row_begin, int32_t row_count);
+int htm_sp_planes_check(htm_handle *h, int64_t out[2]);
 
 int htm_step(htm_handle *h, const uint32_t *packed_input, int32_t learning);
 int htm_sp_step(htm_handle *h, const uint32_t *packed_input, int32_t learning);
```
